# tsurumeso/vocal-remover

Hardware: AMD Instinct MI355X
Metric: spectrogram-frames/sec (inference, CascadedNet n_fft=2048) (higher is better)
Workload: dtype f32; 1 GPU; configs[1]: 30 s stereo 44.1 kHz synthetic song, STFT -> 11 crops of 256 frames in one device batch -> predict_mask -> stitch -> mask apply -> iSTFT x2; n_fft=2048, hop=1024, cropsize=256, parallelism=replicas x1 (songs shard, no collective), input_residency=inputs resident in HBM when the timed region starts

## Files before the change

vocal-remover_amd/csrc/conv_mfma.hip:

```cpp
#include <cstdlib>

#include "conv_stage.h"
#include "kernels.h"

namespace vr {

template <int KS, int S, int DH, int DW, int MT, int TH, int TW, int CK, int WAVES_M>
struct ConvCfg {
    static constexpr int KK = KS * KS;
    static constexpr int WAVES_N = 4 / WAVES_M;
    static constexpr int NG = TH * TW / 32;
    static constexpr int WM = MT / 32 / WAVES_M;
    static constexpr int WN = NG / WAVES_N;
    static constexpr int TH_in = (TH - 1) * S + (KS - 1) * DH + 1;
    static constexpr int TW_in = (TW - 1) * S + (KS - 1) * DW + 1;
    static constexpr int TWp = (TW == 16) ? ((TW_in + 15) / 32 * 32 + 16) : ((TW_in + 1) & ~1);
    static constexpr int XS = CK * TH_in * TWp;
    static constexpr int WS = KK * CK * MT;
    static constexpr int STG = StageGeom<TH_in, TW_in>::TAB + StageGeom<TH_in, TW_in>::SCR;
    static constexpr int LDS_BYTES = (XS + WS + STG) * 4;
    static_assert(WM >= 1 && WN >= 1 && WM * WAVES_M * 32 == MT && WN * WAVES_N == NG, "tile split");
    static_assert(XS % 4 == 0, "weight slab must stay 16B aligned");
    static_assert(TWp >= TW_in, "pitch");
};
// ... 247 lines not shown
}

bool ws_pick(const ConvArgs& a, const ConvShape& s, int* MT_out, int* TH_out);
bool thin16_pick(const ConvArgs& a, const ConvShape& s, int* TH);
void thin16_fill_tiling(ConvArgs& a, int TH);
void thin16_launch_conv(const ConvArgs& a, const ConvShape& s, int TH, hipStream_t st);
bool wino_pick(const ConvArgs& a, const ConvShape& s, int* MT_out);
void wino_fill_tiling(ConvArgs& a, int MT);
void wino_launch_conv(const ConvArgs& a, int MT, hipStream_t st);
struct DmaTile { int MT, TH, TW; };
bool dma_pick(const ConvArgs& a, const ConvShape& s, DmaTile* t);
void dma_fill_tiling(ConvArgs& a, const DmaTile& t);
void dma_launch_conv(const ConvArgs& a, const ConvShape& s, const DmaTile& t, hipStream_t st);
void ws_fill_tiling(ConvArgs& a, int MT, int TH);
void ws_launch_conv(const ConvArgs& a, const ConvShape& s, int MT, int TH, hipStream_t st);

void conv_fill_tiling(ConvArgs& a, const ConvShape& s) {
    int wmt, wth;
    int wino_mt, thin_th;
    if (a.w_hi == 0 && thin16_pick(a, s, &thin_th)) { thin16_fill_tiling(a, thin_th); return; }
    X3Tile x3t;
    if (x3_pick(a, s, &x3t)) { x3_fill_tiling(a, x3t); return; }
    int x3d_mt;
    if (x3d_pick(a, s, &x3d_mt)) { x3d_fill_tiling(a, x3d_mt); return; }
    X3Tile x3st;
    if (x3s_pick(a, s, &x3st)) { x3s_fill_tiling(a, x3st); return; }
    if (wino_pick(a, s, &wino_mt)) { wino_fill_tiling(a, wino_mt); return; }
    DmaTile dt;
    if (dma_pick(a, s, &dt)) { dma_fill_tiling(a, dt); return; }
    if (ws_pick(a, s, &wmt, &wth)) { ws_fill_tiling(a, wmt, wth); return; }
    TileChoice t = pick_tile(a, s);
    a.tiles_w = (a.Wout + t.TW - 1) / t.TW;
    a.tiles_h = (a.Hout + t.TH - 1) / t.TH;
    a.npt = a.N * a.tiles_h * a.tiles_w;
    a.nct = a.CoutPad / t.MT;
}

size_t conv_part_count(const ConvArgs& a, const ConvShape& s) {
    ConvArgs b = a;
    conv_fill_tiling(b, s);
    return (size_t)b.npt;
}

template <int KS, int S, int DH, int DW, int MT, int TH, int TW, int CK, int WAVES_M>
static void launch_inst(const ConvArgs& a, hipStream_t st) {
    using Cfg = ConvCfg<KS, S, DH, DW, MT, TH, TW, CK, WAVES_M>;
    auto kern = conv_mfma_kernel<KS, S, DH, DW, MT, TH, TW, CK, WAVES_M>;
    static std::atomic<unsigned long long> attr_done{0};
    ensure_lds_attr(attr_done, reinterpret_cast<const void*>(kern), Cfg::LDS_BYTES);
    const int groups = (a.npt + 7) / 8;
    const int grid = groups * 8 * a.nct;
    VR_LAUNCH(kern, dim3(grid), dim3(256), Cfg::LDS_BYTES, st, a);
    VR_HIP(hipGetLastError());
}

template <int KS, int S, int DH, int DW, int CK>
static void launch_by_tile(const ConvArgs& a, const TileChoice& t, hipStream_t st) {
    if (t.TW == 32) {
        if constexpr (DH == 1 && DW == 1) {
            if (t.MT == 64) launch_inst<KS, S, DH, DW, 64, 8, 32, CK, 1>(a, st);
            else if (t.TH == 16) {
                if constexpr (S == 1) launch_inst<KS, S, DH, DW, 32, 16, 32, CK, 1>(a, st);
                else throw Error(-2, "16x32 tiles are stride-1 only");
            }
            else            launch_inst<KS, S, DH, DW, 32, 8, 32, CK, 1>(a, st);
        } else {
            throw Error(-2, "dilated conv uses TW=16 tiles only");
        }
    } else {
        if (t.MT == 64) launch_inst<KS, S, DH, DW, 64, 16, 16, CK, 1>(a, st);
        else            launch_inst<KS, S, DH, DW, 32, 16, 16, CK, 1>(a, st);
    }
}

double launch_conv(const ConvArgs& a_in, const ConvShape& s, hipStream_t st) {
    ConvArgs a = a_in;
    static const int dbg = getenv("VR_CONV_DBG") ? atoi(getenv("VR_CONV_DBG")) : 0;
    a.dbg = dbg;
    if (a.w_hi > 0) {
        X3Tile x3t;
        VR_CHECK(a.bf16 == 3 && a.nsrc >= 1 && a.nsrc <= 3 && a.w_lo >= 0 && a.w_lo < a.w_hi && !a.part && x3_pick(a, s, &x3t), -2,
                 "conv column window: only conv_x3h (mfma_mode 3, eval) takes one");
    }
    for (int i = 0; i < a.nsrc && i < 3; ++i) {
        const ConvSrc& c = a.src[i];
        VR_CHECK(!(c.up && c.aff1 && c.aff1 != c.aff0 && c.hsplit < c.H), -2, "conv: an upsampled source cannot carry a row-split affine (hsplit)");
    }
    {
        int wmt, wth;
        int wino_mt, thin_th;
        if (a.w_hi == 0 && a.nsrc >= 1 && a.nsrc <= 3 && thin16_pick(a, s, &thin_th)) {
            thin16_fill_tiling(a, thin_th);
            thin16_launch_conv(a, s, thin_th, st);
            return 2.0 * a.N * (double)a.Hout * a.Wout * (double)a.Cout * a.Cin * s.KS * s.KS;
        }
        X3Tile x3t;
        if (a.nsrc >= 1 && a.nsrc <= 3 && x3_pick(a, s, &x3t)) {
            x3_fill_tiling(a, x3t);
            x3_launch_conv(a, x3t, st);
            return 2.0 * a.N * (double)a.Hout * a.Wout * (double)a.Cout * a.Cin * s.KS * s.KS;
        }
        int x3d_mt;
        if (a.nsrc >= 1 && a.nsrc <= 3 && x3d_pick(a, s, &x3d_mt)) {
            x3d_fill_tiling(a, x3d_mt);
            x3d_launch_conv(a, s, x3d_mt, st);
            return 2.0 * a.N * (double)a.Hout * a.Wout * (double)a.Cout * a.Cin * s.KS * s.KS;
        }
        X3Tile x3st;
        if (x3s_pick(a, s, &x3st)) {
            x3s_fill_tiling(a, x3st);
            x3s_launch_conv(a, x3st, st);
            return 2.0 * a.N * (double)a.Hout * a.Wout * (double)a.Cout * a.Cin * s.KS * s.KS;
        }
        if (a.nsrc >= 1 && a.nsrc <= 3 && wino_pick(a, s, &wino_mt)) {
            wino_fill_tiling(a, wino_mt);
            wino_launch_conv(a, wino_mt, st);
            return 2.0 * a.N * (double)a.Hout * a.Wout * (double)a.Cout * a.Cin * s.KS * s.KS;
        }
        DmaTile dt;
        if (dma_pick(a, s, &dt)) {
            VR_CHECK(a.nsrc >= 1 && a.nsrc <= 3, -2, "conv takes 1..3 sources");
            dma_fill_tiling(a, dt);
            dma_launch_conv(a, s, dt, st);
            return 2.0 * a.N * (double)a.Hout * a.Wout * (double)a.Cout * a.Cin * s.KS * s.KS;
        }
        VR_CHECK(a.tapmask == 0, -2, "a tap-masked conv needs the LDS-DMA kernel (conv_dma_eligible)");
        if (ws_pick(a, s, &wmt, &wth)) {
            VR_CHECK(a.nsrc >= 1 && a.nsrc <= 3, -2, "conv takes 1..3 sources");
            ws_fill_tiling(a, wmt, wth);
            ws_launch_conv(a, s, wmt, wth, st);
            return 2.0 * a.N * (double)a.Hout * a.Wout * (double)a.Cout * a.Cin * s.KS * s.KS;
        }
    }
    conv_fill_tiling(a, s);
    TileChoice t = pick_tile(a, s);
    VR_CHECK(a.CoutPad % t.MT == 0 && a.CoutPad % 32 == 0, -2, "CoutPad must be a multiple of the cout tile");
    VR_CHECK(a.nsrc >= 1 && a.nsrc <= 3, -2, "conv takes 1..3 sources");
    if (s.KS == 1) {
        VR_CHECK(s.stride == 1 && s.dil_h == 1 && s.dil_w == 1, -2, "1x1 conv: stride/dilation must be 1");
        launch_by_tile<1, 1, 1, 1, 32>(a, t, st);
    } else if (s.KS == 3 && s.stride == 1 && s.dil_h == 1 && s.dil_w == 1) {
        launch_by_tile<3, 1, 1, 1, 8>(a, t, st);
    } else if (s.KS == 3 && s.stride == 2 && s.dil_h == 1 && s.dil_w == 1) {
        launch_by_tile<3, 2, 1, 1, 4>(a, t, st);
    } else if (s.KS == 3 && s.stride == 1 && s.dil_h == 4 && s.dil_w == 2) {
        launch_by_tile<3, 1, 4, 2, 4>(a, t, st);
    } else if (s.KS == 3 && s.stride == 1 && s.dil_h == 8 && s.dil_w == 4) {
        launch_by_tile<3, 1, 8, 4, 4>(a, t, st);
    } else if (s.KS == 3 && s.stride == 1 && s.dil_h == 12 && s.dil_w == 6) {
        launch_by_tile<3, 1, 12, 6, 4>(a, t, st);
    } else {
        throw Error(-2, "unsupported conv shape (kernel/stride/dilation)");
    }
    return 2.0 * a.N * (double)a.Hout * a.Wout * (double)a.Cout * a.Cin * s.KS * s.KS;
}

}
```

vocal-remover_amd/csrc/conv_x3h.hip:

```cpp
#include <cstdlib>
#include <type_traits>

#include "conv_epilogue.h"
#include "conv_stage.h"
#include "kernels.h"
#include "lds_dma.h"
#include "x3h_common.h"

namespace vr {

template <int MT, int TH, bool UP = true>
struct X3hCfg {
    static constexpr int TW = 32, CK = 8, KK = 9;
    static constexpr int TH_in = TH + 2, PW = TW + 2;
    static constexpr int NSLOT = TH_in * PW;
    static constexpr int NPASS = (NSLOT + 255) / 256;
    static constexpr int WM = MT / 32, WN = TH / 4;
    static constexpr int PLANE = NSLOT * 16;
    static constexpr int P_BYTES = 2 * PLANE;
    static constexpr int NWP = KK * 2 * MT;
    static constexpr int W_BYTES = NWP * 16;
    static constexpr int NWPASS = (NWP + 255) / 256;
    static constexpr int LROWS = TH / 2 + 3, LW = 20, LSLOT = LROWS * LW;
    static constexpr int L_OFF = P_BYTES + 2 * W_BYTES;
    static constexpr int L_BYTES = UP ? CK * LSLOT * 4 : 0;
    static constexpr int E_OFF = L_OFF + L_BYTES;
    static constexpr int M_OFF = E_OFF + 4 * MT * 4;
    static constexpr int LDS_BYTES = M_OFF + 16;
    static constexpr int OCC = (MT == 32 && TH == 8) ? 3 : 2;
    static constexpr int NXL = 8 * NPASS, NWMIN = (NWP / 64) / 4;
    static constexpr int NG = 14;
    static_assert(TH % 4 == 0 && MT % 32 == 0 && LDS_BYTES <= 80 * 1024 && 2 * NXL + NWMIN < 64 && NXL <= 30 && LSLOT <= 256, "tile");
};

__device__ long long g_x3h_trace[4 * 4 * 6 * 8];
void x3h_trace_read(long long* host, int n) {
    VR_HIP(hipMemcpyFromSymbol(host, HIP_SYMBOL(g_x3h_trace), sizeof(long long) * (size_t)(n < 768 ? n : 768)));
}
void x3h_trace_clear() {
    static long long zeros[768] = {0};
    VR_HIP(hipMemcpyToSymbol(HIP_SYMBOL(g_x3h_trace), zeros, sizeof zeros));
}

template <int MT, int TH, bool UP, bool HI, bool TRACE = false>
__global__ __launch_bounds__(256, (X3hCfg<MT, TH>::OCC + (HI ? 1 : 0))) void conv_x3h_kernel(const ConvArgs a) {
    using Cfg = X3hCfg<MT, TH, UP>;
    constexpr int TW = Cfg::TW, KK = Cfg::KK, PW = Cfg::PW, NSLOT = Cfg::NSLOT, NPASS = Cfg::NPASS, WM = Cfg::WM, WN = Cfg::WN,
                  PLANE = Cfg::PLANE, NWP = Cfg::NWP, NWPASS = Cfg::NWPASS;
    extern __shared__ __attribute__((aligned(16))) char smem_x3h[];
    char* const Pb = smem_x3h;

    const int id = blockIdx.x;
    const int xcd = id & 7;
    const int rr = id >> 3;
    const int ct = rr % a.nct;
    const int per_xcd = (a.npt + 7) >> 3;
    const int pt = (a.dbg & 16) ? (rr / a.nct) * 8 + xcd : xcd * per_xcd + rr / a.nct;
    if (pt >= a.npt) return;
    const int tiles_per_img = a.tiles_h * a.tiles_w;
    const int n = pt / tiles_per_img;
    const int trem = pt - n * tiles_per_img;
    const int h0 = (trem / a.tiles_w) * TH;
    const int w0 = (a.wt0 + trem % a.tiles_w) * TW;
    const int co0 = ct * MT;
    const int tid = threadIdx.x;
    const int lane = tid & 63;
    const int wave = __builtin_amdgcn_readfirstlane(tid >> 6);
    const int nchunk = (a.Cin + 7) >> 3;
    const unsigned lds0 = (unsigned)(size_t)smem_x3h;
    const int dbg = a.dbg & 15;
    const bool prio = (a.dbg & 32) != 0;
    const int trace_wg = TRACE ? (int)blockIdx.x - (int)(gridDim.x / 2) : -1;
    auto stamp = [&](int k, int point) {
        if (TRACE && trace_wg >= 0 && trace_wg < 4 && k >= 2 && k < 8) {
            const long long t = __builtin_readcyclecounter();
            if (lane == 0) g_x3h_trace[((trace_wg * 4 + wave) * 6 + (k - 2)) * 8 + point] = t;
        }
    };

    auto pixel_offset = [&](int p, unsigned sH4) -> int {
        const int s = p * 256 + tid;
        const int r = s / PW, c = s - r * PW;
        const int hi = h0 - 1 + r, wi = w0 - 1 + c;
        const bool ok = s < NSLOT && hi >= 0 && hi < a.Hin && wi >= 0 && wi < a.Win;
        return ok ? (int)((unsigned)hi * sH4 + (unsigned)(wi * 4)) : (int)0x80000000u;
    };
    const ConvSrc& us = a.src[0].up ? a.src[0] : (a.src[1].up ? a.src[1] : a.src[2]);
    constexpr bool any_up = UP;
    int lrow = 0, lcol4 = 0;
    int lidx[NPASS], lstep[NPASS];
    float lh[NPASS], lw_[NPASS];
    if (any_up) {
        const int lr0 = (int)(us.rh * (float)(h0 > 0 ? h0 - 1 : 0)), lc0 = (int)(us.rw * (float)(w0 > 0 ? w0 - 1 : 0));
        const int lr = lr0 + tid / Cfg::LW, lc = lc0 + tid % Cfg::LW;
        const bool lok = tid < Cfg::LSLOT && lr < us.H && lc < us.W;
        lrow = lok ? lr : 0;
        lcol4 = lok ? lc * 4 : (int)0x80000000u;
#pragma unroll
        for (int p = 0; p < NPASS; ++p) {
            const int s = p * 256 + tid;
            const int r = s / PW, c = s - r * PW;
            const int hi = h0 - 1 + r, wi = w0 - 1 + c;
            const bool ok = s < NSLOT && hi >= 0 && hi < a.Hin && wi >= 0 && wi < a.Win;
            const float h1r = us.rh * (float)(ok ? hi : 0), w1r = us.rw * (float)(ok ? wi : 0);
            const int h1 = (int)h1r, w1 = (int)w1r;
            lidx[p] = ok ? ((h1 - lr0) * Cfg::LW + (w1 - lc0)) * 32 : -1;
            const int rs = (h1 + 1 < us.H && h1 + 1 - lr0 < Cfg::LROWS) ? Cfg::LW * 32 : 0;
            const int cs = (w1 + 1 < us.W && w1 + 1 - lc0 < Cfg::LW) ? 32 : 0;
            lstep[p] = (rs << 16) | cs;
            lh[p] = h1r - (float)h1;
            lw_[p] = w1r - (float)w1;
        }
    }
    unsigned woff0;
    {
        const int q = wave * 64 + lane;
        const int m = q % MT, tp = q / MT;
        woff0 = (unsigned)((tp * a.CoutPad + m) * 16);
    }
    const unsigned wstep = (unsigned)((256 / MT) * a.CoutPad * 16);
    const long long wchunk_bytes = (long long)KK * 2 * a.CoutPad * 16;
    auto issue_w = [&](int k) {
        const char* wb = static_cast<const char*>(a.x3w) + k * wchunk_bytes + (long long)co0 * 16;
        const i32x4 wr = make_rsrc(reinterpret_cast<const float*>(wb), (unsigned)(wchunk_bytes - (long long)co0 * 16));
        const unsigned ws_b = lds0 + (unsigned)(Cfg::P_BYTES + (k & 1) * Cfg::W_BYTES);
#pragma unroll
        for (int i = 0; i < NWPASS; ++i) {
            const int pp = wave + 4 * i;
            if ((pp + 1) * 64 <= NWP) dma16s(ws_b + pp * 1024, woff0, wr, (unsigned)i * wstep);
// ... 71 lines not shown
    };
    auto read_max_exp = [&]() -> int {
        const vr_i32x4 mm = *reinterpret_cast<const vr_i32x4*>(smem_x3h + Cfg::M_OFF);
        const int w = max(max(mm[0], mm[1]), max(mm[2], mm[3]));
        return __builtin_amdgcn_readfirstlane(w) >> 23;
    };
    auto convert = [&](auto par) {
        constexpr int PAR = decltype(par)::value;
#pragma unroll
        for (int p = 0; p < NPASS; ++p) {
            const int s = p * 256 + tid;
            if ((p + 1) * 256 <= NSLOT || s < NSLOT) {
                vr_i32x4 ph, pl;
                if (upm[PAR] != 0u) {
                    const char* lq = smem_x3h + Cfg::L_OFF + (lidx[p] >= 0 ? lidx[p] : 0);
                    const int rs = lstep[p] >> 16, cs = lstep[p] & 0xffff;
                    const float h1l = lh[p], h0l = 1.f - h1l, w1l = lw_[p], w0l = 1.f - w1l;
                    if (upm[PAR] == 0xFFu) {
                        vr_f32x4h nb[4][2];
#pragma unroll
                        for (int q4 = 0; q4 < 4; ++q4)
#pragma unroll
                            for (int hf = 0; hf < 2; ++hf)
                                nb[q4][hf] = *reinterpret_cast<const vr_f32x4h*>(lq + (q4 >> 1) * rs + (q4 & 1) * cs + hf * 16);
#pragma unroll
                        for (int cl = 0; cl < 8; ++cl) {
                            const float v00 = nb[0][cl >> 2][cl & 3], v01 = nb[1][cl >> 2][cl & 3], v10 = nb[2][cl >> 2][cl & 3], v11 = nb[3][cl >> 2][cl & 3];
                            const float v = h0l * (w0l * v00 + w1l * v01) + h1l * (w0l * v10 + w1l * v11);
                            xr[PAR][p][cl] = lidx[p] >= 0 ? v : 0.f;
                        }
                    } else {
#pragma unroll
                        for (int cl = 0; cl < 8; ++cl) {
                            if ((upm[PAR] >> cl) & 1u) {
                                const char* q = lq + cl * 4;
                                const float v00 = *reinterpret_cast<const float*>(q), v01 = *reinterpret_cast<const float*>(q + cs),
                                            v10 = *reinterpret_cast<const float*>(q + rs), v11 = *reinterpret_cast<const float*>(q + rs + cs);
                                const float v = h0l * (w0l * v00 + w1l * v01) + h1l * (w0l * v10 + w1l * v11);
                                xr[PAR][p][cl] = lidx[p] >= 0 ? v : 0.f;
                            }
                        }
                    }
                }
#pragma unroll
                for (int j = 0; j < 4; ++j) {
                    int h, l;
                    split2h_pair(xr[PAR][p][2 * j], xr[PAR][p][2 * j + 1], psc, h, l);
                    ph[j] = h; pl[j] = l;
                }
                char* q = Pb + s * 16;
                *reinterpret_cast<vr_i32x4*>(q) = ph;
                *reinterpret_cast<vr_i32x4*>(q + PLANE) = pl;
            }
        }
    };

    const int khalf = lane >> 5, l31 = lane & 31;
    const int bq = (wave * WN * PW + l31) * 16;
    const int bX = bq + khalf * PLANE, bY1 = bq + khalf * 16, bY2 = bq + khalf * (PW - 2) * 16;
    const int aX = l31 * 16, aY = (MT + l31 + khalf * 2 * MT) * 16;

    f32x16 acc[WM][WN];
#pragma unroll
    for (int mi = 0; mi < WM; ++mi)
#pragma unroll
        for (int ni = 0; ni < WN; ++ni)
#pragma unroll
            for (int r = 0; r < 16; ++r) acc[mi][ni][r] = 0.f;

    using P0 = std::integral_constant<int, 0>;
    using P1 = std::integral_constant<int, 1>;
    float ecv[4];
    {
        const int ec = co0 + (tid & (MT - 1));
        const int ecc = ec < a.Cout ? ec : a.Cout - 1;
        const i32x4 rb = make_rsrc(a.bias, a.bias ? 0x7FFFFFF0u : 0u);
        const i32x4 re = make_rsrc(a.epi, a.epi ? 0x7FFFFFF0u : 0u);
        const i32x4 rw = make_rsrc(reinterpret_cast<const float*>(static_cast<const char*>(a.x3w) + nchunk * wchunk_bytes), 0x7FFFFFF0u);
        ecv[0] = x3h_load(rb, ecc * 4);
        ecv[1] = x3h_load(re, ecc * 8);
        ecv[2] = x3h_load(re, ecc * 8 + 4);
        ecv[3] = x3h_load(rw, ec * 4);
    }
    auto follow = [&](int e, bool first) {
        const int need = 140 - (e < 14 ? 14 : e);
        shlo = (first || need < shlo) ? need : shlo;
        int nsh = sh;
        if (first || need < sh - 1) nsh = need;
        else if (need > sh + 12) {
            nsh = need < sh + 64 ? need : sh + 64;
            nsh = nsh < shlo + 64 ? nsh : shlo + 64;
            nsh = nsh > sh ? nsh : sh;
        }
        if (nsh != sh) {
            if (!first) {
                const int d = nsh - sh;
                const float f = d < -126 ? 0.f : x3h_pow2(d);
#pragma unroll
                for (int mi = 0; mi < WM; ++mi)
#pragma unroll
                    for (int ni = 0; ni < WN; ++ni)
#pragma unroll
                        for (int r = 0; r < 16; ++r) acc[mi][ni][r] *= f;
            }
            sh = nsh;
            psc = x3h_pow2(sh);
        }
    };
#pragma unroll
    for (int cl = 0; cl < 8; ++cl) load_channel(0, cl, P0{});
    issue_w(0);
#pragma unroll
    for (int cl = 0; cl < 8; ++cl) load_channel(1, cl, P1{});
    wait_pixels(P0{}, std::integral_constant<int, Cfg::NXL + Cfg::NWMIN>{});
    asm volatile("; landed %0 %1 %2 %3" : "+v"(ecv[0]), "+v"(ecv[1]), "+v"(ecv[2]), "+v"(ecv[3]));
    if (tid < MT) {
        float* E = reinterpret_cast<float*>(smem_x3h + Cfg::E_OFF);
        E[tid] = ecv[0];
        E[MT + tid] = a.epi ? ecv[1] : 1.f;
        E[2 * MT + tid] = a.epi ? ecv[2] : 0.f;
        E[3 * MT + tid] = ecv[3];
    }
    post_max(P0{});
    if (any_up) stage_lowres(P0{});
    lds_barrier();
    follow(read_max_exp(), true);
    convert(P0{});
    asm volatile("s_waitcnt vmcnt(%0) lgkmcnt(0)" :: "n"(Cfg::NXL) : "memory");
    __builtin_amdgcn_s_barrier();
    asm volatile("" ::: "memory");

    auto chunk = [&](int k, auto par) {
        constexpr int PAR = decltype(par)::value;
        const bool more = k + 1 < nchunk;
        stamp(k, 0);
        {
            const char* Wb = smem_x3h + Cfg::P_BYTES + PAR * Cfg::W_BYTES;
            vr_f16x8 A[2][WM], B[2][WN];
            auto read_group = [&](int g, int buf) {
                const bool isY = g == 13 || (g < 12 && g % 3 == 2);
                const int t = g >= 12 ? 8 : 2 * (g / 3) + (g % 3 == 1 ? 1 : 0);
                const int ty = t / 3, tx = t % 3;
#pragma unroll
                for (int mi = 0; mi < WM; ++mi) {
                    const char* q = Wb + (t * 2 * MT + mi * 32) * 16;
                    if (!isY) A[buf][mi] = *reinterpret_cast<const vr_f16x8*>(q + aX);
                    else if (t < 8) A[buf][mi] = *reinterpret_cast<const vr_f16x8*>(q + aY);
                    else {
                        const vr_i32x4 v = *reinterpret_cast<const vr_i32x4*>(q + aX + MT * 16);
                        vr_i32x4 z;
#pragma unroll
                        for (int j = 0; j < 4; ++j) z[j] = khalf ? 0 : v[j];
                        A[buf][mi] = __builtin_bit_cast(vr_f16x8, z);
                    }
                }
#pragma unroll
                for (int ni = 0; ni < WN; ++ni) {
                    const int o = ((ni + ty) * PW + tx) * 16;
                    if (!isY) B[buf][ni] = *reinterpret_cast<const vr_f16x8*>(Pb + bX + o);
                    else if (t == 8) B[buf][ni] = *reinterpret_cast<const vr_f16x8*>(Pb + bq + o);
                    else if (t == 2) B[buf][ni] = *reinterpret_cast<const vr_f16x8*>(Pb + bY2 + o);
                    else B[buf][ni] = *reinterpret_cast<const vr_f16x8*>(Pb + bY1 + o);
                }
            };
            auto mfma_group = [&](int buf) {
#pragma unroll
                for (int mi = 0; mi < WM; ++mi)
#pragma unroll
                    for (int ni = 0; ni < WN; ++ni) acc[mi][ni] = mfma_f16x16(A[buf][mi], B[buf][ni], acc[mi][ni]);
            };
            read_group(0, 0);
            if (prio) __builtin_amdgcn_s_setprio(1);
#pragma unroll
            for (int g = 0; g < Cfg::NG; ++g) {
                const int cur = g & 1;
                if (g + 1 < Cfg::NG) read_group(g + 1, cur ^ 1);
                if (more) {
                    if (g == 0) issue_w(k + 1);
                    if (g >= 1 && g <= 4) { load_channel(k + 2, 2 * g - 2, par); load_channel(k + 2, 2 * g - 1, par); }
                }
                __builtin_amdgcn_sched_barrier(0);
                mfma_group(cur);
                __builtin_amdgcn_sched_barrier(0);
            }
            if (prio) __builtin_amdgcn_s_setprio(0);
        }
        stamp(k, 1);
        if (more) {
            using Q = std::integral_constant<int, PAR ^ 1>;
            wait_pixels(Q{}, std::integral_constant<int, Cfg::NXL + Cfg::NWMIN>{});
            stamp(k, 2);
            post_max(Q{});
            if (any_up) stage_lowres(Q{});
            stamp(k, 3);
            lds_barrier();
            stamp(k, 4);
            follow(read_max_exp(), false);
            if (dbg != 3) convert(Q{});
            stamp(k, 5);
            asm volatile("s_waitcnt vmcnt(%0) lgkmcnt(0)" :: "n"(Cfg::NXL) : "memory");
            stamp(k, 6);
            __builtin_amdgcn_s_barrier();
            asm volatile("" ::: "memory");
            stamp(k, 7);
        }
    };
    for (int k = 0; k < nchunk; k += 2) {
        chunk(k, P0{});
        if (k + 1 < nchunk) chunk(k + 1, P1{});
    }
    asm volatile("s_waitcnt vmcnt(0)" ::: "memory");

    if (dbg == 4) return;
    {
        const float fo = x3h_pow2(-sh);
        const float* Wi = reinterpret_cast<const float*>(smem_x3h + Cfg::E_OFF) + 3 * MT;
#pragma unroll
        for (int mi = 0; mi < WM; ++mi)
#pragma unroll
            for (int rq = 0; rq < 4; ++rq) {
                const vr_f32x4h wi = *reinterpret_cast<const vr_f32x4h*>(Wi + mi * 32 + 8 * rq + 4 * khalf);
#pragma unroll
                for (int ni = 0; ni < WN; ++ni)
#pragma unroll
                    for (int j = 0; j < 4; ++j) acc[mi][ni][rq * 4 + j] = (acc[mi][ni][rq * 4 + j] * fo) * wi[j];
            }
    }
    {
        int hon[WN], won[WN];
#pragma unroll
        for (int ni = 0; ni < WN; ++ni) { hon[ni] = h0 + wave * WN + ni; won[ni] = w0 + l31; }
        epi_store<MT, WM, WN>(VR_EPI_ARGS(a), acc, reinterpret_cast<const float*>(smem_x3h + Cfg::E_OFF), n, co0, khalf,
                              h0 + TH <= a.Hout && w0 + TW <= a.Wout, hon, won);
    }
    if (a.part) {
        __syncthreads();
        float* red = reinterpret_cast<float*>(smem_x3h);
#pragma unroll
        for (int mi = 0; mi < WM; ++mi) {
#pragma unroll
            for (int r = 0; r < 16; ++r) {
                float s1 = 0.f, s2 = 0.f;
#pragma unroll
                for (int ni = 0; ni < WN; ++ni) {
                    const int ho = h0 + wave * WN + ni, wo = w0 + l31;
                    if (ho < a.Hout && wo < a.Wout) {
                        const float v = acc[mi][ni][r];
                        s1 += v;
                        s2 = fmaf(v, v, s2);
                    }
                }
                s1 = half_wave_sum_dpp(s1);
                s2 = half_wave_sum_dpp(s2);
                if (l31 == 16) {
                    const int m = mi * 32 + (r & 3) + 8 * (r >> 2) + 4 * khalf;
                    red[(wave * MT + m) * 2 + 0] = s1;
                    red[(wave * MT + m) * 2 + 1] = s2;
                }
            }
        }
        __syncthreads();
        if (tid < MT) {
            float s1 = 0.f, s2 = 0.f;
#pragma unroll
            for (int w = 0; w < 4; ++w) {
                s1 += red[(w * MT + tid) * 2 + 0];
                s2 += red[(w * MT + tid) * 2 + 1];
            }
            const int co = co0 + tid;
            if (co < a.Cout) {
                a.part[((long long)pt * a.Cout + co) * 2 + 0] = s1;
                a.part[((long long)pt * a.Cout + co) * 2 + 1] = s2;
            }
        }
    }
}

__device__ __forceinline__ float* x3h_tail(void* o, int Cin, int KK, int CoutPad) {
    return reinterpret_cast<float*>(static_cast<char*>(o) + (size_t)((Cin + 7) / 8) * KK * 2 * CoutPad * 16);
}
__device__ __forceinline__ void x3h_wscale_block(const float* __restrict__ w, void* o, int Cin, int KK, int CoutPad, int cb) {
    __shared__ float red[8][32];
    if (cb * 32 >= CoutPad) return;
    const int c = threadIdx.x & 31, g = threadIdx.x >> 5, co = cb * 32 + c;
    const int rows = Cin * KK;
    float m = 0.f;
    for (int r = g; r < rows; r += 8) m = fmaxf(m, fabsf(w[(long long)r * CoutPad + co]));
    red[g][c] = m;
    __syncthreads();
    if (g == 0) {
#pragma unroll
        for (int j = 1; j < 8; ++j) m = fmaxf(m, red[j][c]);
        int e = __float_as_int(m) >> 23;
        e = e < 15 ? 15 : (e > 254 ? 254 : e);
        float* t = x3h_tail(o, Cin, KK, CoutPad);
        t[co] = __int_as_float((e - 14) << 23);
        t[CoutPad + co] = __int_as_float((268 - e) << 23);
    }
}
__device__ __forceinline__ void x3h_weights_elem(const float* __restrict__ w, void* o, int Cin, int KK, int CoutPad, long long gid) {
    const int cin8 = (Cin + 7) / 8 * 8;
    if (gid >= (long long)cin8 * KK * CoutPad) return;
    const int co = (int)(gid % CoutPad);
    const int t = (int)((gid / CoutPad) % KK);
    const int ci = (int)(gid / ((long long)CoutPad * KK));
    const float sc = x3h_tail(o, Cin, KK, CoutPad)[CoutPad + co];
    const float v = ci < Cin ? w[((long long)ci * KK + t) * CoutPad + co] : 0.f;
    const _Float16 h1 = (_Float16)(v * sc);
    const _Float16 h2 = (_Float16)fmaf(v, sc, -(float)h1);
    _Float16* q = static_cast<_Float16*>(o) + ((((long long)(ci >> 3) * KK + t) * 2) * CoutPad + co) * 8 + (ci & 7);
    q[0] = h1;
    q[(long long)CoutPad * 8] = h2;
}
__global__ void x3h_wscale_kernel(const float* __restrict__ w, void* o, int Cin, int KK, int CoutPad) {
    x3h_wscale_block(w, o, Cin, KK, CoutPad, blockIdx.x);
}
__global__ void x3h_weights_kernel(const float* __restrict__ w, void* o, int Cin, int KK, int CoutPad) {
    x3h_weights_elem(w, o, Cin, KK, CoutPad, (long long)blockIdx.x * blockDim.x + threadIdx.x);
}
__global__ void x3h_wscale_batched_kernel(const X3WDesc* __restrict__ d) {
    const X3WDesc e = d[blockIdx.y];
    x3h_wscale_block(e.w, e.o, e.Cin, e.KK, e.CoutPad, blockIdx.x);
}
__global__ void x3h_weights_batched_kernel(const X3WDesc* __restrict__ d) {
    const X3WDesc e = d[blockIdx.y];
    x3h_weights_elem(e.w, e.o, e.Cin, e.KK, e.CoutPad, (long long)blockIdx.x * blockDim.x + threadIdx.x);
}

void launch_x3h_weights(const float* w, void* o, int Cin, int KK, int CoutPad, hipStream_t st) {
    const long long n = (long long)((Cin + 7) / 8 * 8) * KK * CoutPad;
    VR_LAUNCH(x3h_wscale_kernel, dim3((unsigned)((CoutPad + 31) / 32)), dim3(256), 0, st, w, o, Cin, KK, CoutPad);
    VR_LAUNCH(x3h_weights_kernel, dim3((unsigned)((n + 255) / 256)), dim3(256), 0, st, w, o, Cin, KK, CoutPad);
    VR_HIP(hipGetLastError());
}
void launch_x3h_weights_batched(const X3WDesc* d_descs, int n, long long max_elems, int max_cout_pad, hipStream_t st) {
    if (n <= 0) return;
    VR_LAUNCH(x3h_wscale_batched_kernel, dim3((unsigned)((max_cout_pad + 31) / 32), (unsigned)n), dim3(256), 0, st, d_descs);
    VR_LAUNCH(x3h_weights_batched_kernel, dim3((unsigned)((max_elems + 255) / 256), (unsigned)n), dim3(256), 0, st, d_descs);
    VR_HIP(hipGetLastError());
}

template <int MT, int TH, bool UP, bool HI, bool TRACE = false>
static void x3h_launch_up(const ConvArgs& a, hipStream_t st) {
    using Cfg = X3hCfg<MT, TH, UP>;
    auto kern = conv_x3h_kernel<MT, TH, UP, HI, TRACE>;
    static std::atomic<unsigned long long> attr_done{0};
    ensure_lds_attr(attr_done, reinterpret_cast<const void*>(kern), Cfg::LDS_BYTES);
    const int groups = (a.npt + 7) / 8;
    VR_LAUNCH(kern, dim3(groups * 8 * a.nct), dim3(256), Cfg::LDS_BYTES, st, a);
    VR_HIP(hipGetLastError());
}

template <int MT, int TH>
static void x3h_launch(const ConvArgs& a, hipStream_t st) {
    static const int hi = [] { const char* e = getenv("VR_X3H_HI"); return e ? atoi(e) : 0; }();
    if (a.dbg & 64) {
        if (a.src[0].up | a.src[1].up | a.src[2].up) x3h_launch_up<MT, TH, true, false, true>(a, st);
        else x3h_launch_up<MT, TH, false, false, true>(a, st);
        return;
    }
    if (a.src[0].up | a.src[1].up | a.src[2].up) x3h_launch_up<MT, TH, true, false>(a, st);
    else if (hi && TH == 8) x3h_launch_up<MT, TH, false, (TH == 8)>(a, st);
    else x3h_launch_up<MT, TH, false, false>(a, st);
}

void x3h_launch_conv(const ConvArgs& a, const X3Tile& t, hipStream_t st) {
    if (t.MT == 64) x3h_launch<64, 8>(a, st);
    else if (t.TH == 16) x3h_launch<32, 16>(a, st);
    else x3h_launch<32, 8>(a, st);
}

}
```

vocal-remover_amd/csrc/debug.hip:

```cpp
#include <cmath>
#include <cstdlib>
#include <cstring>
#include <memory>
#include <string>
#include <vector>

#include "model.h"

namespace vr {

namespace {

struct DevBuf {
    float* p = nullptr;
    size_t n = 0;
    DevBuf() = default;
    explicit DevBuf(size_t n_) : n(n_) {
        VR_HIP(hipMalloc(&p, (n ? n : 1) * sizeof(float)));
        VR_HIP(hipMemset(p, 0, (n ? n : 1) * sizeof(float)));
        VR_HIP(hipStreamSynchronize(nullptr));
    }
    DevBuf(const float* host, size_t n_) : n(n_) {
        VR_HIP(hipMalloc(&p, (n ? n : 1) * sizeof(float)));
        if (host && n) VR_HIP(hipMemcpy(p, host, n * sizeof(float), hipMemcpyHostToDevice));
// ... 245 lines not shown
    ConvArgs a{};
    a.nsrc = nsrc; a.N = N; a.Cout = Cout; a.CoutPad = (Cout + 31) / 32 * 32;
    a.w_lo = (int)dims[8]; a.w_hi = (int)dims[9]; a.d1 = (int)dims[10]; a.d2 = (int)dims[11];
    a.bf16 = mfma_mode;
    a.pad_h = KS == 1 ? 0 : dh; a.pad_w = KS == 1 ? 0 : dw;
    std::vector<std::unique_ptr<DevBuf>> keep;
    auto upload = [&](const float* host, size_t n) { keep.emplace_back(new DevBuf(host, n)); return keep.back()->p; };
    int Cin = 0;
    const ConvSrc* ups = nullptr;
    for (int i = 0; i < nsrc; ++i) {
        const int64_t* d = dims + 12 + 10 * i;
        const float* const* si = in + 3 + 4 * i;
        Tensor t;
        t.N = N; t.C = (int)d[0]; t.H = (int)d[1]; t.W = (int)d[2];
        const bool up = d[3] != 0;
        t.hsplit = (int)d[4];
        const size_t floats = (size_t)d[5];
        t.sN = d[7]; t.sC = d[8]; t.sH = d[9];
        VR_CHECK(si[0] && view_fits(d[6], t.sN, t.sC, t.sH, N, t.C, t.H, t.W, floats), -2, who + "a source view leaves its buffer");
        t.p = upload(si[0], floats) + d[6];
        t.slope = fp[1 + i];
        if (si[1]) t.aff0 = upload(si[1], (size_t)t.C * 2);
        if (si[2]) t.aff1 = upload(si[2], (size_t)t.C * 2);
        if (si[3]) t.post = upload(si[3], (size_t)N * t.C);
        a.src[i] = make_src(t, up, 0);
        const int vh = up ? 2 * t.H : t.H, vw = up ? 2 * t.W : t.W;
        if (i == 0) { a.Hin = vh; a.Win = vw; }
        VR_CHECK(vh == a.Hin && vw == a.Win, -2, who + "the sources must share the input size");
        if (up && ups) VR_CHECK(ups->H == t.H && ups->W == t.W && ups->sH == t.sH, -2, who + "upsampled sources must share H, W and row stride");
        if (up) ups = &a.src[i];
        Cin += t.C;
        if (i == 0) a.c1 = Cin;
        if (i <= 1) a.c2 = Cin;
    }
    a.Cin = Cin;
    a.Hout = a.Hin; a.Wout = a.Win;
    const int KK = KS * KS;
    std::vector<float> wk((size_t)Cin * KK * a.CoutPad, 0.f);
    for (int co = 0; co < Cout; ++co)
        for (int ci = 0; ci < Cin; ++ci)
            for (int k = 0; k < KK; ++k) wk[((size_t)ci * KK + k) * a.CoutPad + co] = in[0][((size_t)co * Cin + ci) * KK + k];
    DevBuf dwk(wk.data(), wk.size());
    a.w = dwk.p;
    if (in[1]) a.bias = upload(in[1], (size_t)Cout);
    if (in[2]) { a.epi = upload(in[2], (size_t)Cout * 2); a.epi_slope = fp[0]; }
    DebugWeightForms wf;
    debug_weight_forms(dwk.p, Cin, KS, 1, dh, dw, a.CoutPad, a.Win, transformed, a, wf);
    std::vector<std::unique_ptr<GuardedBuf>> dst(3);
    const int c1 = a.d1 < Cout ? a.d1 : Cout, c2 = a.d2 < Cout ? a.d2 : Cout;
    VR_CHECK(0 <= c1 && c1 <= c2, -2, who + "need 0 <= d1 <= d2");
    const int seg_c[3] = {c1, c2 - c1, Cout - c2};
    for (int i = 0; i < ndst; ++i) {
        const int64_t* d = dims + 12 + 10 * nsrc + 7 * i;
        const float* host = in[3 + 4 * nsrc + i];
        if (!d[0]) continue;
        VR_CHECK(host && out[i], -2, who + "a present destination needs its buffer, in and out");
        VR_CHECK(seg_c[i] == 0 || view_fits(d[3], d[4], d[5], d[6], N, seg_c[i], a.Hout, a.Wout, (size_t)d[2]), -2,
                 who + "a destination view leaves its buffer");
        dst[i].reset(new GuardedBuf(host, (size_t)d[2]));
        a.dst[i] = ConvDst{dst[i]->p() + d[3], d[4], d[5], d[6], d[1] != 0 ? 1 : 0, 0};
    }
    const ConvShape shp{KS, 1, dh, dw};
    size_t npt = 0;
    std::unique_ptr<DevBuf> part;
    if (want_part) { npt = conv_part_count(a, shp); part.reset(new DevBuf(npt * Cout * 2)); a.part = part->p; }
    launch_conv(a, shp, stream);
    VR_HIP(hipStreamSynchronize(stream));
    for (int i = 0; i < ndst; ++i)
        if (dst[i]) {
            VR_CHECK(dst[i]->intact(), -3, who + "the launch stored outside a destination's buffer");
            dst[i]->download(out[i]);
        }
    if (want_part) {
        std::vector<float> ph(npt * Cout * 2);
        part->download(ph.data());
        for (int c = 0; c < Cout; ++c) {
            double s1 = 0, s2 = 0;
            for (size_t i = 0; i < npt; ++i) { s1 += ph[(i * Cout + c) * 2]; s2 += ph[(i * Cout + c) * 2 + 1]; }
            out[ndst][2 * c] = (float)s1; out[ndst][2 * c + 1] = (float)s2;
        }
    }
}

void Model::debug_wgrad_launch(const int64_t* dims, int ndims, const float* fp, int nfp, const float* const* in, int nin, float* const* out,
                               int nout) {
    const std::string who = "vr_debug_kernel(wgrad_launch): ";
    VR_CHECK(ndims >= 13 && nfp >= 3 && nin >= 2 && nout >= 2, -2, who + "too few arguments");
    const int nsrc = (int)dims[0], N = (int)dims[1], Cout = (int)dims[2], KS = (int)dims[3], stride = (int)dims[4];
    const int dh = (int)dims[5], dw = (int)dims[6], flags = (int)dims[7];
    const bool batch_as_h = flags & 1, accumulate = flags & 2, defer = flags & 4, twice = flags & 8, accumulate2 = flags & 16;
    VR_CHECK(nsrc >= 1 && nsrc <= 3 && N >= 1 && Cout >= 1 && (KS == 1 || KS == 3) && (stride == 1 || stride == 2) && dh >= 1 && dw >= 1, -2,
             who + "1..3 sources, a 1x1 or 3x3 kernel, stride 1 or 2");
    VR_CHECK(ndims >= 13 + 10 * nsrc && nin >= 2 + 4 * nsrc, -2, who + "too few arguments");
    VR_CHECK(in[0] && in[1] && out[0] && out[1], -2, who + "missing dz, gradient or an output");
    WgradArgs w{};
    ConvArgs& a = w.in;
    a.nsrc = nsrc; a.Cout = Cout; a.CoutPad = (Cout + 31) / 32 * 32;
    a.d1 = a.d2 = 1 << 30;
    a.pad_h = KS == 1 ? 0 : dh; a.pad_w = KS == 1 ? 0 : dw;
    std::vector<std::unique_ptr<DevBuf>> keep;
    auto upload = [&](const float* host, size_t n) { keep.emplace_back(new DevBuf(host, n)); return keep.back()->p; };
    int Cin = 0, Hin = 0, Win = 0;
    const ConvSrc* ups = nullptr;
    for (int i = 0; i < nsrc; ++i) {
        const int64_t* d = dims + 13 + 10 * i;
        const float* const* si = in + 2 + 4 * i;
        Tensor t;
        t.N = N; t.C = (int)d[0]; t.H = (int)d[1]; t.W = (int)d[2];
        const bool up = d[3] != 0;
        t.hsplit = (int)d[4];
        const size_t floats = (size_t)d[5];
        t.sN = d[7]; t.sC = d[8]; t.sH = d[9];
        VR_CHECK(si[0] && view_fits(d[6], t.sN, t.sC, t.sH, N, t.C, t.H, t.W, floats), -2, who + "a source view leaves its buffer");
        t.p = upload(si[0], floats) + d[6];
        t.slope = fp[i];
        if (si[1]) t.aff0 = upload(si[1], (size_t)t.C * 2);
        if (si[2]) t.aff1 = upload(si[2], (size_t)t.C * 2);
        if (si[3]) t.post = upload(si[3], (size_t)N * t.C);
        a.src[i] = make_src(t, up, 0);
        const int vh = up ? 2 * t.H : t.H, vw = up ? 2 * t.W : t.W;
        if (i == 0) { Hin = vh; Win = vw; }
        VR_CHECK(vh == Hin && vw == Win, -2, who + "the sources must share the input size");
        if (up && ups) VR_CHECK(ups->H == t.H && ups->W == t.W && ups->sH == t.sH, -2, who + "upsampled sources must share H, W and row stride");
        if (up) ups = &a.src[i];
        Cin += t.C;
        if (i == 0) a.c1 = Cin;
        if (i <= 1) a.c2 = Cin;
    }
    a.Cin = Cin;
    if (nsrc < 2) a.c1 = Cin;
    if (nsrc < 3) a.c2 = Cin;
    const int Hout0 = (Hin + 2 * a.pad_h - dh * (KS - 1) - 1) / stride + 1, Wout = (Win + 2 * a.pad_w - dw * (KS - 1) - 1) / stride + 1;
    VR_CHECK(Hout0 >= 1 && Wout >= 1, -2, who + "empty output");
    const size_t zfloats = (size_t)dims[8];
    VR_CHECK(view_fits(dims[9], dims[10], dims[11], dims[12], N, Cout, Hout0, Wout, zfloats), -2, who + "the dz view leaves its buffer");
    DevBuf dz(in[0], zfloats);
    w.dz = dz.p + dims[9];
    int Nk = N;
    if (batch_as_h) {
        VR_CHECK(KS == 1 && Hin == 1, -2, who + "batch-as-rows view needs a 1x1 conv on H=1 input");
        for (int i = 0; i < nsrc; ++i) {
            VR_CHECK(!a.src[i].post && !a.src[i].up, -2, who + "batch-as-rows: unsupported source flags");
            a.src[i].sH = a.src[i].sN; a.src[i].sN = 0; a.src[i].H = N;
        }
        Hin = N; Nk = 1;
        w.zN = 0; w.zC = dims[11]; w.zH = dims[10];
    } else {
        w.zN = dims[10]; w.zC = dims[11]; w.zH = dims[12];
    }
    a.N = Nk; a.Hin = Hin; a.Win = Win;
    a.Hout = (Hin + 2 * a.pad_h - dh * (KS - 1) - 1) / stride + 1; a.Wout = Wout;
    w.Cout = Cout; w.CoutPad = a.CoutPad;
    w.allow_wino = train_wino ? 1 : 0;
    w.bf16 = mfma_mode;
    const ConvShape shp{KS, stride, dh, dw};
    WgradArgs pl = w;
    {
        int CB = 0, MT = 0;
        wgrad_choose(pl, shp, &CB, &MT);
    }
    const size_t gfloats = (size_t)Cin * KS * KS * a.CoutPad, sfloats = wgrad_scratch_floats(w, shp);
    VR_CHECK((size_t)pl.P * (size_t)pl.part_stride <= sfloats, -4, who + "the plan's slabs exceed wgrad_scratch_floats");
    GuardedBuf grad(in[1], gfloats);
    const std::vector<float> nans(sfloats, std::nanf(""));
    GuardedBuf scratch(nans.data(), sfloats), scratch2(twice ? nans.data() : nullptr, twice ? sfloats : 0);
    w.part = scratch.p();
// ... 93 lines not shown
    debug_dgrad_weight_forms(P, KS, stride, dh, dw, forms);
    struct WsRestore {
        Model* m; Arena saved;
        ~WsRestore() { m->ws = saved; m->dry = false; }
    } ws_restore{this, ws};
    ws.dry = true; ws.base = nullptr; ws.off = 0; ws.peak = 0; dry = true;
    bwd_conv_dgrad(r, f);
    dry = false;
    const size_t wfloats = (ws.peak + 3) / 4;
    const std::vector<float> nans(wfloats, std::nanf(""));
    GuardedBuf wsbuf(nans.data(), wfloats);
    ws = Arena{};
    ws.base = reinterpret_cast<char*>(wsbuf.p()); ws.cap = wfloats * 4;
    int path = DG_NONE;
    try {
        path = bwd_conv_dgrad(r, f);
    } catch (...) {
        (void)hipStreamSynchronize(stream);
        for (int i = 0; i < nsrc; ++i) grads[i]->download(out[i]);
        throw;
    }
    VR_HIP(hipStreamSynchronize(stream));
    bool intact = wsbuf.intact();
    for (int i = 0; i < nsrc; ++i) intact = intact && grads[i]->intact();
    VR_CHECK(intact, -3, who + "the launch stored outside a gradient buffer or the workspace");
    for (int i = 0; i < nsrc; ++i) grads[i]->download(out[i]);
    const int64_t info[4] = {path, (int64_t)wfloats, 0, 0};
    std::memcpy(out[nsrc], info, sizeof info);
}

void Model::debug_wgrad_reduce(const int64_t* dims, int ndims, const float* const* in, int nin, float* const* out, int nout) {
    const std::string who = "vr_debug_kernel(wgrad_reduce): ";
    VR_CHECK(ndims >= 1, -2, who + "too few arguments");
    const int nd = (int)dims[0];
    VR_CHECK(nd >= 1 && nd <= 128 && ndims >= 1 + 6 * nd && nin >= 2 * nd && nout >= 2 * nd + 1, -2, who + "1..128 descriptors, six dims each");
    std::vector<std::unique_ptr<DevBuf>> slabs;
    std::vector<std::unique_ptr<GuardedBuf>> o_imm, o_bat;
    std::vector<WgReduceDesc> descs;
    for (int j = 0; j < nd; ++j) {
        const int64_t* d = dims + 1 + 6 * j;
        const long long P = d[0], n = d[1], stride = d[2], floats = d[4], off = d[5];
        VR_CHECK(P >= 1 && n >= 1 && stride >= n && off >= 0 && off + n <= floats, -2, who + "need P, n >= 1, stride >= n and the output inside its buffer");
        VR_CHECK(in[2 * j] && in[2 * j + 1] && out[2 * j] && out[2 * j + 1] && out[2 * nd], -2, who + "missing buffer");
        slabs.emplace_back(new DevBuf(in[2 * j], (size_t)(P * stride)));
        o_imm.emplace_back(new GuardedBuf(in[2 * j + 1], (size_t)floats));
        o_bat.emplace_back(new GuardedBuf(in[2 * j + 1], (size_t)floats));
        descs.push_back(WgReduceDesc{slabs.back()->p, stride, o_bat.back()->p() + off, n, (int)P, d[3] != 0 ? 1 : 0, 0});
    }
    for (int j = 0; j < nd; ++j) {
        const WgReduceDesc& d = descs[j];
        launch_wgrad_reduce(d.part, d.stride, d.P, o_imm[j]->p() + dims[1 + 6 * j + 5], d.n, d.accumulate, stream);
    }
    const int vec = wgrad_reduce_vec(descs.data(), nd);
    wred_host = descs;
    flush_wgrad_sums();
    VR_HIP(hipStreamSynchronize(stream));
    for (int j = 0; j < nd; ++j) {
        VR_CHECK(o_imm[j]->intact() && o_bat[j]->intact(), -3, who + "a slab sum stored outside its output buffer");
        o_imm[j]->download(out[2 * j]);
        o_bat[j]->download(out[2 * j + 1]);
    }
    out[2 * nd][0] = (float)vec;
}

void Model::debug_kernel(const std::string& name, const int64_t* dims, int ndims, const float* fp, int nfp,
                         const float* const* in, int nin, float* const* out, int nout) {
    DeviceGuard dev_guard(device);
    auto need = [&](int nd, int nf, int ni, int no) {
        VR_CHECK(ndims >= nd && nfp >= nf && nin >= ni && nout >= no, -2, "vr_debug_kernel(" + name + "): too few arguments");
    };
    hipStream_t st = stream;
    if (name == "x3h_trace") {
        need(1, 0, 0, dims[0] ? 1 : 0);
        VR_HIP(hipDeviceSynchronize());
        if (!dims[0]) { x3h_trace_clear(); return; }
        long long raw[768];
        x3h_trace_read(raw, 768);
        long long lo = 0;
        for (long long v : raw) if (v && (!lo || v < lo)) lo = v;
        for (int i = 0; i < 768; ++i) out[0][i] = raw[i] ? (float)(raw[i] - lo) : -1.f;
        return;
    }
    if (name == "conv_launch") { debug_conv_launch(dims, ndims, fp, nfp, in, nin, out, nout); return; }
    if (name == "wgrad_launch") { debug_wgrad_launch(dims, ndims, fp, nfp, in, nin, out, nout); return; }
    if (name == "wgrad_reduce") { debug_wgrad_reduce(dims, ndims, in, nin, out, nout); return; }
    if (name == "dgrad_launch") { debug_dgrad_launch(dims, ndims, in, nin, out, nout); return; }
    if (name == "tensor_pass") { debug_tensor_pass(dims, ndims, fp, nfp, in, nin, out, nout); return; }
    if (name == "weight_forms") { debug_weight_form_launch(dims, ndims, in, nin, out, nout); return; }
    if (name == "layer_forms") { debug_layer_forms(dims, ndims, out, nout); return; }
    if (name == "bn_backward") {
        need(4, 3, 7, 6);
        const int N = (int)dims[0], C = (int)dims[1], H = (int)dims[2], W = (int)dims[3];
        const bool view = ndims >= 10;
        const long long off = view ? dims[5] : 0, sH = view ? dims[8] : W, sC = view ? dims[7] : (long long)H * W, sN = view ? dims[6] : sC * C;
        const size_t n = view ? (size_t)dims[4] : (size_t)N * C * H * W;
        const int aff_bcast = view && dims[9] != 0 ? 1 : 0;
        VR_CHECK(N >= 1 && C >= 1 && H >= 1 && W >= 1, -2, "bn_backward: empty tensor");
        VR_CHECK(view_fits(off, sN, sC, sH, N, C, H, W, n), -2, "bn_backward: the view leaves its buffer");
        VR_CHECK(!aff_bcast || C == 1, -2, "bn_backward: a broadcast affine table belongs to a single-channel BatchNorm");
        DevBuf z(in[0], n), gamma(in[2], C), beta(in[3], C), rm(in[5], C), rv(in[6], C);
        GuardedBuf g(in[1], n);
        DevBuf post(in[4], in[4] ? (size_t)N * C : 0);
        std::vector<float> part((size_t)C * 2);
        for (int c = 0; c < C; ++c) {
            double s1 = 0, s2 = 0;
            for (int b = 0; b < N; ++b)
                for (int h = 0; h < H; ++h) {
                    const float* q = in[0] + off + b * sN + c * sC + h * sH;
                    for (int i = 0; i < W; ++i) { s1 += q[i]; s2 += (double)q[i] * q[i]; }
                }
            part[2 * c] = (float)s1; part[2 * c + 1] = (float)s2;
        }
        const int bcast_rows = aff_bcast ? 8 : 0;
        DevBuf dpart(part.data(), part.size()), aff((size_t)(aff_bcast ? bcast_rows : C) * 2), smean(C), sinv(C), dgamma(C), dbeta(C);
        BNFinalizeArgs f{};
        f.part = dpart.p; f.nparts = 1; f.pstride = C * 2; f.count = (double)N * H * W;
        f.w = gamma.p; f.b = beta.p; f.rm = rm.p; f.rv = rv.p; f.affine = aff.p; f.save_mean = smean.p; f.save_invstd = sinv.p;
        f.C = C; f.eps = fp[1]; f.momentum = fp[2]; f.broadcast = bcast_rows;
        launch_bn_finalize(f, st);
        BnBwdArgs a{};
        a.g = g.p() + off; a.z = z.p + off; a.N = N; a.C = C; a.H = H; a.W = W; a.sH = sH; a.sC = sC; a.sN = sN;
        a.aff = aff.p; a.aff_bcast = aff_bcast; a.slope = fp[0]; a.post = in[4] ? post.p : nullptr;
        a.gamma = gamma.p; a.save_mean = smean.p; a.save_invstd = sinv.p; a.dgamma = dgamma.p; a.dbeta = dbeta.p; a.acc_grads = 1;
        DevBuf coef((size_t)C * 3), bpart((size_t)bn_bwd_chunks(a) * C * 2);
        a.coef = coef.p; a.part = bpart.p;
        launch_bn_bwd(a, st);
        VR_HIP(hipStreamSynchronize(st));
        VR_CHECK(g.intact(), -3, "bn_backward: a store outside the gradient's buffer");
        g.download(out[0]); dgamma.download(out[1]); dbeta.download(out[2]); rm.download(out[4]); rv.download(out[5]);
        if (out[3]) VR_HIP(hipMemcpy(out[3], aff.p, (size_t)C * 2 * sizeof(float), hipMemcpyDeviceToHost));
    } else if (name == "lstm") {
        const int flags = ndims >= 4 ? (int)dims[3] : 0;
        const bool infer = flags & 1, bwd_only = flags & 2;
        need(3, 0, infer ? 3 : 4, infer ? 1 : 4);
        const int N = (int)dims[0], T = (int)dims[1], H = (int)dims[2], G = 4 * H;
        VR_CHECK(N > 0 && T > 0 && H > 0, -2, "lstm: N, T, H must be positive");
        DevBuf gx(in[0], (size_t)N * 2 * G * T), wf(in[1], (size_t)G * H), wr(in[2], (size_t)G * H), h((size_t)N * 2 * H * T);
        if (infer) {
            launch_bilstm(gx.p, wf.p, wr.p, h.p, N, T, H, st);
            VR_HIP(hipStreamSynchronize(st));
            h.download(out[0]);
            return;
        }
        DevBuf dh(in[3], (size_t)N * 2 * H * T), save((size_t)N * 2 * T * 5 * H), dgx((size_t)N * 2 * G * T);
        const float* f0 = nin >= 5 ? in[4] : nullptr;
        const float* r0 = nin >= 6 ? in[5] : nullptr;
        std::vector<float> zeros(f0 && r0 ? 0 : (size_t)G * H, 0.f);
        DevBuf dwf(f0 ? f0 : zeros.data(), (size_t)G * H), dwr(r0 ? r0 : zeros.data(), (size_t)G * H);
        if (!bwd_only) launch_bilstm_train(gx.p, wf.p, wr.p, h.p, save.p, N, T, H, st);
        launch_bilstm_bwd(dh.p, save.p, wf.p, wr.p, dgx.p, N, T, H, st);
        DevBuf wpart(lstm_whh_grad_scratch_floats(N, H));
        launch_lstm_whh_grad(dgx.p, h.p, dwf.p, dwr.p, N, T, H, 1, wpart.p, st);
        VR_HIP(hipStreamSynchronize(st));
        h.download(out[0]); dgx.download(out[1]); dwf.download(out[2]); dwr.download(out[3]);
    } else if (name == "upsample") {
        need(4, 0, 2, 2);
        const int N = (int)dims[0], C = (int)dims[1], H = (int)dims[2], W = (int)dims[3];
        const size_t n = (size_t)N * C * H * W;
        const bool view = ndims >= 10;
        const long long off = view ? dims[5] : 0, gN = view ? dims[6] : (long long)C * H * W, gC = view ? dims[7] : (long long)H * W, gH = view ? dims[8] : W;
        const size_t gfloats = view ? (size_t)dims[4] : n;
        VR_CHECK(N >= 1 && C >= 1 && H >= 1 && W >= 1, -2, "upsample: empty tensor");
        VR_CHECK(!view || (nin >= 3 && in[2]), -2, "upsample: a strided gradient needs its backing buffer");
        VR_CHECK(view_fits(off, gN, gC, gH, N, C, H, W, gfloats), -2, "upsample: the gradient view leaves its buffer");
        const std::vector<float> zeros(view ? 0 : n, 0.f);
        DevBuf x(in[0], n), dhi(in[1], 4 * n), up(4 * n);
// ... 416 lines not shown
```

vocal-remover_amd/csrc/kernels.h:

```cpp
#pragma once
#include "vr_common.h"

namespace vr {

struct HeadDst {
    float* p;
    long long dN, dC, dH;
    int w_lo, w_hi;
    int pad_rows;
    float* const* items;
    const int* item_pitch;
};
void launch_head_sigmoid(const Tensor& x, const float* w , const HeadDst& d, hipStream_t st);
void launch_head_complex(const Tensor& x, const float* w , const HeadDst& d, hipStream_t st);
int launch_squeeze_conv(const Tensor& x, const float* w , float* out, float* part, bool dry, hipStream_t st,
                        const float* epi = nullptr);

void launch_avgpool_h(const Tensor& x, float* out, hipStream_t st);

struct BNFoldDesc { const float *w, *b, *rm, *rv; float* affine; int C; int bcast; };
void launch_bn_fold_eval(const BNFoldDesc* d_descs, int ndesc, int maxC, float eps, hipStream_t st);
struct BNFinalizeArgs {
    const float* part; int nparts; int pstride;
    double count;
    const float *w, *b; float *rm, *rv;
    float* affine; float* save_mean; float* save_invstd;
    int C; float eps, momentum;
    int broadcast;
};
void launch_bn_finalize(const BNFinalizeArgs& a, hipStream_t st);

void launch_rows_affine_relu(const float* x, float* out, const float* aff, int N, int R, int W, hipStream_t st);

void launch_add(const float* a, const float* b, float* out, int n, hipStream_t st);

void launch_materialize(const Tensor& x, float* out, hipStream_t st);
struct AugDesc { float coef, coef_mix, lam; int flags; };
void launch_augment(const float2* X, const float2* Y, const float2* Xi, const float2* Yi, const AugDesc* desc, const float* rw,
                    int B, int T, int bins, float* Xmag, float* Ymag, bool out_complex, hipStream_t st);
struct AugCrops { const float2 *X, *y, *X_mix, *y_mix; };
void launch_augment_resident(const AugCrops* table, const AugDesc* desc, const float* rw, int B, int T, int bins, float* Xmag,
                             float* Ymag, bool out_complex, hipStream_t st);
bool thin16_pick(const ConvArgs& a, const ConvShape& s, int* TH);
void thin16_fill_tiling(ConvArgs& a, int TH);
void thin16_launch_conv(const ConvArgs& a, const ConvShape& s, int TH, hipStream_t st);
bool s2d_fused_eligible(const ConvArgs& a);
void launch_s2d_fused(const ConvArgs& a, hipStream_t st);
struct S2WDesc { const float* w; float* wc; int Cin, Cout, CoutPad, CinPad; };
void launch_s2_class_weights(const S2WDesc* d_descs, int n, long long max_elems, hipStream_t st);
void launch_wino_weights(const float* w, float* u, int Cin, int CoutPad, hipStream_t st);
struct WinoWDesc { const float* w; void* u; int Cin, CoutPad; };
void launch_wino_weights_batched(const WinoWDesc* d_descs, int n, long long max_elems, bool split6, hipStream_t st);
size_t wino_weights6_bytes(int Cin, int CoutPad);
void launch_wino_weights6(const float* w, void* u6, int Cin, int CoutPad, hipStream_t st);
struct X3Tile { int MT, TH; };
struct X3WDesc { const float* w; void* o; int Cin, KK, CoutPad; };
bool x3_pick(const ConvArgs& a, const ConvShape& s, X3Tile* t);
void x3_fill_tiling(ConvArgs& a, const X3Tile& t);
void x3_launch_conv(const ConvArgs& a, const X3Tile& t, hipStream_t st);
size_t x3_weights_bytes(int Cin, int KK, int CoutPad);
void launch_x3_weights(const float* w, void* o, int Cin, int KK, int CoutPad, hipStream_t st);
void launch_x3_weights_batched(const X3WDesc* d_descs, int n, long long max_elems, hipStream_t st);
void x3h_launch_conv(const ConvArgs& a, const X3Tile& t, hipStream_t st);
void x3h_trace_read(long long* host, int n);
void x3h_trace_clear();
void launch_x3h_weights(const float* w, void* o, int Cin, int KK, int CoutPad, hipStream_t st);
void launch_x3h_weights_batched(const X3WDesc* d_descs, int n, long long max_elems, int max_cout_pad, hipStream_t st);
bool x3d_pick(const ConvArgs& a, const ConvShape& s, int* MT);
void x3d_fill_tiling(ConvArgs& a, int MT);
void x3d_launch_conv(const ConvArgs& a, const ConvShape& s, int MT, hipStream_t st);
bool x3d_aspp_eligible(const ConvArgs* c4, const ConvShape* s4);
void x3d_launch_aspp(const ConvArgs* c4, hipStream_t st);
bool x3s_pick(const ConvArgs& a, const ConvShape& s, X3Tile* t);
void x3s_fill_tiling(ConvArgs& a, const X3Tile& t);
void x3s_launch_conv(const ConvArgs& a, const X3Tile& t, hipStream_t st);
void launch_upsample2x(const Tensor& x, float* out, hipStream_t st);

void launch_bilstm(const float* gx, const float* whh_f, const float* whh_r, float* out,
                   int N, int T, int H, hipStream_t st);

void launch_bilstm_train(const float* gx, const float* whh_f, const float* whh_r, float* out, float* save,
                         int N, int T, int H, hipStream_t st);
void launch_bilstm_bwd(const float* dh, const float* save, const float* whh_f, const float* whh_r, float* dgx,
                       int N, int T, int H, hipStream_t st);
size_t lstm_whh_grad_scratch_floats(int N, int H);
void launch_lstm_whh_grad(const float* dgx, const float* hout, float* dwhh_f, float* dwhh_r, int N, int T, int H,
                          int accumulate, float* part, hipStream_t st);

struct BnBwdArgs {
    float* g;
    const float* z;
    int N, C, H, W;
    long long sN, sC, sH;
    const float* aff;
    int aff_bcast;
    float slope;
    const float* post;
    const float *gamma, *save_mean, *save_invstd;
    float *dgamma, *dbeta;
    int acc_grads;
    float* coef;
    float* part;
};
int bn_bwd_chunks(const BnBwdArgs& a);
void launch_bn_bwd(const BnBwdArgs& a, hipStream_t st);

void launch_upsample_bwd(const float* dhi, int N, int C, int H, int W, float* glo, long long gN, long long gC,
                         long long gH, int accumulate, hipStream_t st);
void launch_sum_h(const float* d, int N, int C, int H, int W, float* out, hipStream_t st);
void launch_avgpool_bwd(const float* gp, float* g, int N, int C, int H, int W, long long sN, long long sC, long long sH,
                        int accumulate, hipStream_t st);
void launch_thin_dgrad(const Tensor& x, int CO, const float* w, const float* dz, float* g, int accumulate, hipStream_t st);
int thin_wgrad_blocks(const Tensor& x);
void launch_thin_wgrad(const Tensor& x, int CO, const float* dz, float* part, float* dw, int accumulate, hipStream_t st);
void launch_reduce_rows(const float* part, long long stride, int P, float* out, long long n, int accumulate, float scale,
                        hipStream_t st);
int head_loss_blocks(const Tensor& x);
void launch_head_loss(const Tensor& x, const float* w, const float* X, const float* Y, int bins, float gscale,
                      float* dlogit, float* mask_out, float* loss_part, float* loss_out, float loss_scale, hipStream_t st);
void launch_head_bwd(const float* dmask, const float* mask, int N, int H, int W, int bins, float* dlogit, hipStream_t st);
void launch_head_loss_complex(const Tensor& x, const float* w, const float* X, const float* Y, int bins, float gscale,
                              float* dlogit, float* mask_out, float* loss_part, float* loss_out, float loss_scale, hipStream_t st);
void launch_head_bwd_complex(const Tensor& x, const float* w, const float* dmask, int bins, float* dlogit, hipStream_t st);
struct MagL1 {};
void launch_head_mag_l1(const Tensor& x, const float* w, const float* X, const float* Y, int bins, float* mask_out, float* loss_part,
                        float* loss_out, float loss_scale, hipStream_t st);
struct FlipDesc { const float* w; float* wt; int Cin, Cout, KK, CinPad, CoutPad; };
void launch_flip_transpose(const FlipDesc* d_descs, int n, hipStream_t st);
void launch_adam(float* p, const float* g, float* m, float* v, long long n, double lr, double b1, double b2, double eps,
                 long long step, double gscale, hipStream_t st);
void launch_channel_sum(const float* d, int N, int C, int W, float* out, int accumulate, hipStream_t st);
void launch_f32_to_bf16(const float* x, unsigned short* y, long long n, hipStream_t st);
void launch_bf16_to_f32(const unsigned short* x, float* y, long long n, hipStream_t st);

void launch_mul_crop(const float* x, float* m, bool cplx, long long rows, int T, int Wm, int off, hipStream_t st);
int l1_crop_blocks();
enum L1CropForm { L1_CROP_REAL = 0, L1_CROP_COMPLEX = 1, L1_CROP_MAG = 2 };
void launch_l1_crop(L1CropForm form, const float* pred, const float* y, long long rows, int T, int Wm, int off, float* part, float* loss,
                    hipStream_t st);

struct FFTPlan { int n_fft; int log2n; float2* twiddle; float* window; };
void launch_stft(const FFTPlan& pl, const float* wave, long long L, int hop, int T, float2* spec, hipStream_t st);
void launch_istft(const FFTPlan& pl, const float2* spec, int hop, int T, float* frames, float* wave, hipStream_t st);
bool istft_masked_available(const FFTPlan& pl, int hop);
void launch_istft_masked(const FFTPlan& pl, const float2* spec, int hop, int T, const float* mask_a, int Wa, const float* mask_b,
                         int Wb, int shift, const float* wgt, int which, float* wave, hipStream_t st);
// ... 161 lines not shown
```

vocal-remover_amd/csrc/model.h:

```cpp
#pragma once
#include <chrono>
#include <deque>
#include <functional>
#include <map>
#include <memory>
#include <string>
#include <vector>

#include "kernels.h"

namespace vr {

struct Arena {
    char* base = nullptr;
    size_t cap = 0, off = 0, peak = 0;
    bool dry = false;
    void* alloc(size_t bytes) {
        const size_t a = (off + 255) & ~size_t(255);
        off = a + bytes;
        if (off > peak) peak = off;
        if (dry) return reinterpret_cast<void*>(uintptr_t(256));
        if (off > cap) throw Error(-4, "workspace arena overflow (planning bug)");
        return base + a;
    }
// ... 97 lines not shown
    long long bytes = 0;
    ResidentSet(int device, int bins);
    ~ResidentSet();
    ResidentSet(const ResidentSet&) = delete;
    ResidentSet& operator=(const ResidentSet&) = delete;
    int add(const float* X, const float* y, long long rows);
private:
    static constexpr size_t kPiece = size_t(8) << 20;
    hipStream_t up = nullptr;
    char* stage[2] = {nullptr, nullptr};
    hipEvent_t drained[2] = {nullptr, nullptr};
    void upload(float2* dst, const float* src, size_t n_bytes);
};

struct HeadScratch {
    float *dlogit, *lpart, *wpart;
    float *mask, *dmask, *wave[3], *part, *table;
};
struct TrainHead {
    int kind; bool cplx;
    const float *w, *X, *Y; int bins;
    float* mask;
    float* loss;
    float loss_scale, grad_scale, sdr_scale;
    float* g; int g_acc; float* dw; int dw_acc;
};
template <class ALLOC>
HeadScratch head_scratch(ALLOC&& allocf, const FFTPlan& pl, int hop, const Tensor& f3, int kind, bool cplx, int bins) {
    const int CO = cplx ? 4 : 2;
    HeadScratch s{};
    s.dlogit = allocf((size_t)f3.N * CO * f3.H * f3.W);
    s.lpart = allocf((size_t)head_loss_blocks(f3));
    s.wpart = allocf((size_t)thin_wgrad_blocks(f3) * CO * f3.C);
    if (kind == 0) return s;
    const WaveTermFloats wf = wave_term_floats(pl, hop, kind, f3.N * 2, f3.W);
    s.mask = allocf((size_t)f3.N * 2 * bins * f3.W * 2);
    s.dmask = allocf((size_t)f3.N * 2 * bins * f3.W * 2);
    for (int i = 0; i < wf.waves; ++i) s.wave[i] = allocf(wf.wave);
    s.part = allocf(wf.part);
    s.table = allocf(wf.table);
    return s;
}
void run_train_head(const FFTPlan& pl, const Tensor& f3, const TrainHead& h, const HeadScratch& s, WaveTable* staging, hipStream_t st);
void launch_head_grads(const Tensor& f3, int CO, const float* w, const float* dlogit, float* wpart, float* g, int g_acc, float* dw,
                       int dw_acc, hipStream_t st);

class Model {
public:
    Model(int device, int n_fft, int hop, int nout, int nout_lstm, bool is_complex = false);
    ~Model();

    int device, n_fft, hop, nout, nout_lstm, max_bin, output_bin, offset = 64;
    bool is_complex = false;
    bool complex_train = false;
    int loss_kind = 0;
    double sdr_weight = 0.01, last_mag_l1 = 0.0, last_sdr = 0.0;
    bool loss_terms_valid = false;
    WaveTable wave_host{};
    double last_y_sdr = 0.0, last_noise_sdr = 0.0, last_alpha = 0.0;
    void set_loss(int kind, double weight);
    float finish_wave_loss(const float* l4);
    float finish_wsdr_loss(const float* l7);
    int nin = 2;
    void need_real_mask(const char* what) const;
    void need_real_mask_train(const char* what) const;

    std::deque<Param> params;
    std::map<std::string, Param*> by_key;
    void set_param(const std::string& key, const void* host, const int64_t* shape, int ndim);
    void get_param(const std::string& key, void* host, int64_t cap_bytes);
    void set_training(bool t);
    bool training = false;
    bool fwd_only = false;
    bool taping() const { return training && !fwd_only; }

    void forward_api(const float* x, bool x_on_device, int B, int T, int mode, float* out, bool out_on_device);

    void validate_api(const float* X, const float* Y, bool on_dev, int B, int T, float* loss_out);
    void debug_kernel(const std::string& name, const int64_t* dims, int ndims, const float* fp, int nfp,
                      const float* const* in, int nin, float* const* out, int nout);

    void debug_conv_launch(const int64_t* dims, int ndims, const float* fp, int nfp, const float* const* in, int nin, float* const* out,
                           int nout);
    void debug_wgrad_launch(const int64_t* dims, int ndims, const float* fp, int nfp, const float* const* in, int nin, float* const* out,
                            int nout);
    void debug_wgrad_reduce(const int64_t* dims, int ndims, const float* const* in, int nin, float* const* out, int nout);
    void debug_dgrad_launch(const int64_t* dims, int ndims, const float* const* in, int nin, float* const* out, int nout);
    void debug_tensor_pass(const int64_t* dims, int ndims, const float* fp, int nfp, const float* const* in, int nin, float* const* out,
                           int nout);
    void debug_weight_form_launch(const int64_t* dims, int ndims, const float* const* in, int nin, float* const* out, int nout);
    void debug_layer_forms(const int64_t* dims, int ndims, float* const* out, int nout);
    void stft_api(const float* wave, bool on_dev, long long L, float* spec, bool spec_on_dev);
    void istft_api(const float* spec, bool on_dev, int T, float* wave, bool wave_on_dev);
    void separate_run(int n_songs, const float* const* in, bool in_on_dev, const int* T, const long long* L, int tta, int batchsize,
                      int cropsize, float* const* y, float* const* v, bool out_on_dev, const int* pcm_channels = nullptr,
                      const int* pcm_fmt = nullptr, bool solo = false, const EvalArgs* eval = nullptr);
    bool pcm_available() const;
    void check_pcm(const void* bytes, int channels, int fmt, const std::string& who) const;
    void stft_pcm_api(const void* bytes, bool on_dev, long long L, int channels, int fmt, float* spec, bool spec_on_dev);
    void istft_pcm16_api(const float* spec, bool on_dev, int T, int16_t* out, bool out_on_dev);
    void run_crop_chunks(int patches, int bs, const std::function<void(int, int)>& run_crops);
    StreamState* stream_open(int cropsize, int batchsize, int flags, double coef_re, double coef_im);
    void stream_push(StreamState& S, const float* wave, bool on_dev, long long n, bool flush, float* y, float* v, bool out_on_dev,
                     long long capacity, long long* n_out);
    void stream_push_many(int n_streams, StreamState* const* S, const float* const* wave, bool on_dev, const long long* n, const int* flush,
                          int batchsize, float* const* y, float* const* v, bool out_on_dev, const long long* capacity, long long* n_out);
    void stream_close(StreamState* S);
    void arena_bytes(long long* staging, long long* workspace) const { *staging = (long long)io.cap; *workspace = (long long)ws.cap; }

    void debug_conv(const float* x, int N, int Cin, int H, int W, const float* w_oihw, int Cout, int KS, int stride,
                    int dh, int dw, int up, const float* aff, float slope, const float* bias, float* out,
                    float* stats_out);
    struct DebugWeightForms {
        float* wino = nullptr;
        void* wino6 = nullptr;
        void* x3w = nullptr;
        DebugWeightForms() = default;
        ~DebugWeightForms() { (void)hipFree(wino); (void)hipFree(wino6); (void)hipFree(x3w); }
        DebugWeightForms(const DebugWeightForms&) = delete;
        DebugWeightForms& operator=(const DebugWeightForms&) = delete;
    };
    void debug_weight_forms(const float* dw_kmajor, int Cin, int KS, int stride, int dh, int dw, int CoutPad, int Win, bool transformed,
                            ConvArgs& a, DebugWeightForms& f);
    bool record_taps = false;
    std::map<std::string, Tensor> taps;
    int64_t get_tap(const std::string& name, float* host, int64_t cap_floats, int64_t* shape4);

    bool profiling = false;
    LaunchProfiler* launch_prof = nullptr;
    std::string profile_report;
    void profile_begin();
    void augment_api(const float* Xc, const float* yc, const float* Xi, const float* yi, const void* desc, const float* rw,
                     int B, int T, int bins, bool in_on_dev, float* Xmag, float* ymag, bool out_on_dev, bool out_complex = false);
    void dataset_batch_api(const ResidentSet& set, const ResidentCrop* crops, const void* desc, const float* rw, int B, int T,
                           float* Xmag, float* ymag, bool out_on_dev, bool out_complex = false);
    char* aug_buf = nullptr; size_t aug_cap = 0;
    void aug_reserve(size_t need);
    bool train_wino = true;
    int mfma_mode = 3;
    bool x3_mode() const { return mfma_mode == 2 || mfma_mode == 3; }
    int default_mfma_mode = 3;
    bool serial = false;
    bool crop_window = true;
    int net_w_lo = 0, net_w_hi = 0;
    void set_option(const std::string& name, int value);
    void reset_adam_state();
    void profile_end(double* conv_ms, double* conv_flops, double* conv_bytes, int* launches);

    hipStream_t stream = nullptr;
    hipStream_t side_stream = nullptr;
    hipEvent_t ev_fork = nullptr, ev_join = nullptr;
    bool band_fork_active = false;
    bool gs_clear_pending = false;
    bool wgrad_on_side = false;
    struct Lane { hipStream_t main = nullptr, side = nullptr; hipEvent_t fork = nullptr, join = nullptr, start = nullptr, done = nullptr; Arena ws; };
    std::vector<Lane> lanes;
    void swap_lane(int i);

private:
    float* p_arena = nullptr; size_t p_floats = 0;
    float* b_arena = nullptr; size_t b_floats = 0;
    Arena ws;
    Arena io;
    void ensure_ws(size_t bytes);
    int plan_B = -1, plan_T = -1; bool plan_training = false; size_t plan_peak = 0;
    void ensure_io(size_t bytes);

    std::deque<BN> bns;
    std::vector<BN*> bn_list;
    std::vector<Conv*> wino_list;
    struct PendingConv { ConvArgs a; ConvShape shp; double flops, bytes; bool stats; BNFinalizeArgs fin; BN* bn; };
    std::vector<PendingConv>* conv_sink = nullptr;
    int x3d_mode = 2;
    int conv_w_lo = 0, conv_w_hi = 0;
    std::vector<Conv*> x3d_list;
    int x3s_mode = x3s_default();
    static int x3s_default() { const char* e = getenv("VR_CONV_X3S"); return (e && atoi(e) == 0) ? 0 : 1; }
    std::vector<Conv*> x3s_list;
    float* wino_arena = nullptr;
    float* winot_arena = nullptr;
    std::map<const Param*, float*> winot_of;
    char* wino6_arena = nullptr;
    char* winot6_arena = nullptr;
    std::map<const Param*, void*> winot6_of;
    char* x3_arena = nullptr;
    char* x3t_arena = nullptr;
    std::map<const Param*, void*> x3t_of;
    std::map<const Param*, void*> x3dt_of;
    std::vector<WgReduceDesc> wred_host, wred_sent;
    WgReduceDesc* wred_dev = nullptr;
    size_t wred_cap = 0;
    void flush_wgrad_sums();
    struct X3Batch { std::vector<X3WDesc> host; X3WDesc* dev = nullptr; long long max_elems = 0; };
    X3Batch xb_fwd, xb_bwd;
    void run_x3_batch(X3Batch& b, std::vector<X3WDesc>& descs);
    static long long x3_batch_max_elems(const std::vector<X3WDesc>& descs);
    static int x3_batch_max_cout_pad(const std::vector<X3WDesc>& descs);
    static long long wino_batch_max_elems(const std::vector<WinoWDesc>& descs, bool split6);
    static long long s2w_batch_max_elems(const std::vector<S2WDesc>& descs);
    void refresh_wino(bool with_dgrad);
    struct WinoBatch { std::vector<WinoWDesc> host; WinoWDesc* dev = nullptr; long long max_elems = 0; };
    WinoBatch wb_fwd, wb_bwd, wb_fwd6, wb_bwd6;
    void run_wino_batch(WinoBatch& b, std::vector<WinoWDesc>& descs, bool split6);
    BNFoldDesc* d_fold = nullptr;
    bool affine_dirty = true;
    void fold_eval_affines();

    BaseNetL nets_[5];
    Conv tail1, tail2;
    Param *out_w = nullptr, *aux_out_w = nullptr;

    FFTPlan plan{};

    Param* add_param(const std::string& key, std::vector<int64_t> shape, ParamKind kind, bool trainable);
    BN* add_bn(const std::string& prefix, int C, int bcast);
    void build_cba(Conv& L, const std::string& prefix, int nin, int nout_, int ks, int stride, int pad_h, int pad_w,
                   int dh, int dw, float slope);
    void build_basenet(BaseNetL& B, const std::string& prefix, int nin, int c, int nin_lstm, int nout_lstm_);
    void finalize_layout();

    struct SrcSpec { Tensor t; bool up = false; int bcastH = 0; float* plain = nullptr; };
    enum TapeKind { TK_CONV, TK_AVGPOOL, TK_SQUEEZE, TK_LSTM, TK_DENSE_ACT };
    struct TapeRec {
        TapeKind kind;
        Conv* L = nullptr;
        std::vector<SrcSpec> srcs;
// ... 2 lines not shown
        bool batch_as_h = false;
        const float* bias = nullptr;
        Param* bias_param = nullptr;
        LSTMMod* M = nullptr;
        Tensor aux;
        float* save = nullptr;
        float* buf0 = nullptr;
        float* buf1 = nullptr;
        int chain = 0;
    };
    std::vector<TapeRec> tape;
    Arena gs;
    std::vector<std::pair<size_t, size_t>> gs_zero, gs_zero_plan;
    std::map<const float*, bool> g_fresh;
    float* galloc(size_t n, bool plain);
    bool g_first(const float* g);
    void clear_gs_zero_ranges(hipStream_t st);
    float* g_arena = nullptr;
    float* m_arena = nullptr; float* v_arena = nullptr;
    float* wt_arena = nullptr; size_t wt_floats = 0;
    FlipDesc* d_flip = nullptr; int n_flip = 0;
    std::map<const Param*, float*> wt_of;
    float* s2w_arena = nullptr;
    std::map<const Param*, float*> s2w_of;
    std::vector<Conv*> s2_list;
    S2WDesc* d_s2w = nullptr;
    long long s2w_max = 0;
    long long adam_step = 0;
    float* grad_of(const Param* p) { return p->grad_override ? p->grad_override : g_arena + (p->dev - p_arena); }
public:
    void debug_conv_bwd(const float* x, int N, int Cin, int H, int W, const float* w_oihw, int Cout, int KS, int stride,
                        int dh, int dw, int up, const float* aff, float slope, const float* dz, float* dx_out,
                        float* dw_out);
private:
    void ensure_train_state();
    void refresh_train_weights();
    template <class F> void plan_train_arenas(F&& dry_run, size_t extra_ws, bool clear_beside);
    void wait_gs_clear();
    void backward();
    void bwd_conv(TapeRec& r);
    enum DgradPath { DG_NONE = 0, DG_STRIDE1 = 1, DG_S2_FUSED = 2, DG_S2_CLASSES = 3, DG_S2_ZINS = 4 };
    int bwd_conv_dgrad(TapeRec& r, const ConvArgs& f);
    struct DebugDgradForms {
        Model* m = nullptr;
        const Param* P = nullptr;
        float *wt = nullptr, *winot = nullptr, *s2w = nullptr;
        void *x3t = nullptr, *flip_desc = nullptr, *s2_desc = nullptr;
        DebugDgradForms() = default;
        ~DebugDgradForms();
        DebugDgradForms(const DebugDgradForms&) = delete;
        DebugDgradForms& operator=(const DebugDgradForms&) = delete;
    };
    void debug_dgrad_weight_forms(const Param& P, int KS, int stride, int dh, int dw, DebugDgradForms& f);
    void bwd_bn_of(const Tensor& out, Conv& L);
    std::vector<float> dropout_host;
    int dropout_mode = 1;
    unsigned long long dropout_seed = 0x5DEECE66Dull;
    unsigned long long train_calls = 0;
    void prepare_dropout(int B);
    float* dropout_buf = nullptr; size_t dropout_cap = 0;
public:
    void train_fwd_bwd_api(const float* X, const float* Y, bool on_dev, int B, int T, int accumulation_steps,
                           float* loss_out, float* mask_out, bool mask_on_dev);
    void forward_train_api(const float* X, bool on_dev, int B, int T, float* mask_out, bool mask_on_dev);
    void backward_api(const float* dmask, bool on_dev);
    bool graph_valid = false; int graph_B = 0, graph_T = 0; Tensor graph_f3; float* graph_mask = nullptr;
    int64_t graph_gen = 0;
    void param_arena(float** ptr, int64_t* numel) { *ptr = p_arena; *numel = (int64_t)p_floats; }
    void mark_params_dirty() { affine_dirty = true; }
    void adam_step_api(double lr, double b1, double b2, double eps, double grad_scale);
    void zero_grad_api();
    void adam_state(float* m_host, float* v_host, int64_t numel, int64_t* step, bool set);
    void get_grad(const std::string& key, float* host, int64_t cap_bytes);
    void set_dropout(int mode, unsigned long long seed, const float* masks, int B);
    void grad_arena(float** ptr, int64_t* numel);
    void comm_init(int rank, int world, const void* id128);
    void comm_destroy();
    void allreduce_grads(int wire_dtype);
    void broadcast_params(int root, bool with_optimizer);
    void* comm = nullptr; int comm_rank = 0, comm_world = 1;
    void* wire_buf = nullptr;
private:
    void build_fwd_args(Conv& L, const std::vector<SrcSpec>& srcs, int N, bool batch_as_h, ConvArgs& a);
    Tensor run_conv(Conv& L, const std::vector<SrcSpec>& srcs, int N, const Tensor* out_view, const float* bias,
                    bool batch_as_h);
    template <class F> void for_each_conv(F&& f);
    std::vector<Conv*> conv_layers();
    Tensor run_basenet(BaseNetL& B, const std::vector<SrcSpec>& in, int N, const Tensor* out_view);
    Tensor run_net_window(const Tensor& x, int w_lo, int w_hi);
    Tensor run_lstm(LSTMMod& M, const Tensor& h);
    SrcSpec upsampled(const Tensor& t);
    Tensor run_net(const Tensor& x);
    Tensor net_input(const float* X, const hipMemcpyKind* copy, int B, int T, const float** xd = nullptr);
    void mask_head(const Tensor& f3, int w_lo, int w_hi, HeadDst d);
    void mask_head(const Tensor& f3, int w_lo, int w_hi, float* out);
    void crop_mask_head(const Tensor& f3, int cropsize, HeadDst d);
    void run_dense_crops(float* dense, int count, int cropsize, const HeadDst& d);
    struct StreamStepIO { const float* blk; long long blk_n, blk_pitch; float *y, *v; long long out_pitch, out_off; };
    struct StreamPart {
        StreamState* S; const float* wave; long long n; bool flush; float *y, *v; long long capacity, need;
        long long at; bool flush_done; float *stage_in, *stage_y, *stage_v; StreamStepIO o;
        std::vector<unsigned long long> st;
    };
    struct StreamStepPlan { StreamSeg seg; StreamSchedule p; int new_frames, segments; bool emit; };
    struct StreamCrop { int entry, pass; long long idx; };
    long long stream_check(const StreamState& S, const std::string& who, const float* wave, long long n, bool flush, const float* y,
                           const float* v, bool out_on_dev, long long capacity) const;
    void stream_run(std::vector<StreamPart>& parts, int bs, bool on_dev, bool out_on_dev);
    StreamStepPlan stream_step_plan(StreamState& S, const StreamStepIO& io_, bool final);
    void stream_step_crops(const StreamState& S, const StreamStepPlan& sp, int entry, std::vector<StreamCrop>& list) const;
    void stream_step_commit(StreamState& S, StreamStepIO& io_, const StreamStepPlan& sp);
    void tap(const std::string& name, const Tensor& t);
    bool dry = false;
    const float* dropout_dev = nullptr;
    void plan_and_reserve(int B, int T, size_t extra_bytes);
    void record_begin(int kind, double flops);
    void record_note(double bytes, const char* tag);
    double conv_alg_bytes(const Conv& L, const ConvArgs& a, int N, bool batch_as_h) const;
    void record_end();
};

}
```

vocal-remover_amd/csrc/model.hip:

```cpp
#include "pcm.h"
#include "model.h"

#include <algorithm>
#include <chrono>
#include <cmath>
#include <cstdlib>
#include <cstring>

namespace vr {

static inline int round_up(int v, int m) { return (v + m - 1) / m * m; }

Param* Model::add_param(const std::string& key, std::vector<int64_t> shape, ParamKind kind, bool trainable) {
    params.emplace_back();
    Param* p = &params.back();
    p->key = key;
    p->shape = std::move(shape);
    p->kind = kind;
    p->trainable = trainable;
    p->numel = 1;
    for (auto d : p->shape) p->numel *= (size_t)d;
    p->dev_numel = p->numel;
    if (kind == PK_CONV) {
        p->Cout = (int)p->shape[0];
// ... 255 lines not shown
}

void Model::get_param(const std::string& key, void* host, int64_t cap_bytes) {
    auto it = by_key.find(key);
    VR_CHECK(it != by_key.end(), -2, "unknown parameter key: " + key);
    Param& p = *it->second;
    DeviceGuard dev_guard(device);
    VR_HIP(hipStreamSynchronize(stream));
    if (p.kind == PK_NBT) {
        VR_CHECK(cap_bytes >= 8, -2, "buffer too small");
        *static_cast<int64_t*>(host) = p.nbt;
        return;
    }
    VR_CHECK((size_t)cap_bytes >= p.numel * sizeof(float), -2, "buffer too small for " + key);
    float* dst = static_cast<float*>(host);
    if (p.kind == PK_CONV) {
        std::vector<float> tmp((size_t)p.Cin * p.KK * p.CoutPad);
        VR_HIP(hipMemcpy(tmp.data(), p.dev, tmp.size() * sizeof(float), hipMemcpyDeviceToHost));
        for (int co = 0; co < p.Cout; ++co)
            for (int ci = 0; ci < p.Cin; ++ci)
                for (int k = 0; k < p.KK; ++k)
                    dst[((size_t)co * p.Cin + ci) * p.KK + k] = tmp[((size_t)ci * p.KK + k) * p.CoutPad + co];
    } else if (p.kind == PK_LSTM_IH) {
        std::vector<float> tmp((size_t)p.Cin * p.Cout);
        VR_HIP(hipMemcpy2D(tmp.data(), (size_t)p.Cout * sizeof(float), p.dev + p.co_off, (size_t)p.CoutPad * sizeof(float),
                           (size_t)p.Cout * sizeof(float), (size_t)p.Cin, hipMemcpyDeviceToHost));
        for (int co = 0; co < p.Cout; ++co)
            for (int ci = 0; ci < p.Cin; ++ci) dst[(size_t)co * p.Cin + ci] = tmp[(size_t)ci * p.Cout + co];
    } else {
        VR_HIP(hipMemcpy(dst, p.dev, p.numel * sizeof(float), hipMemcpyDeviceToHost));
    }
}

void Model::need_real_mask(const char* what) const {
    VR_CHECK(!is_complex || complex_train, -2, std::string(what) + ": this handle predicts a complex mask (is_complex=True); only eval-mode inference "
                              "is supported for it, training is not");
}

void Model::need_real_mask_train(const char* what) const {
    VR_CHECK(!(is_complex && training) || complex_train, -2, std::string(what) + " in training mode: this handle predicts a complex mask "
                                            "(is_complex=True); only eval-mode inference is supported for it, training is not");
}

void Model::set_training(bool t) {
    if (training && !t) affine_dirty = true;
    training = t;
}

void Model::fold_eval_affines() {
    if (!affine_dirty) return;
    int maxC = 1;
    for (BN* b : bn_list) maxC = std::max(maxC, std::max(b->C, b->bcast));
    launch_bn_fold_eval(d_fold, (int)bn_list.size(), maxC, 1e-5f, stream);
    refresh_wino(false);
    for (BaseNetL& B : nets_) {
        LSTMMod& M = B.lstm;
        const int G = 4 * M.hid;
        if (!M.bias_sum) VR_HIP(hipMalloc(reinterpret_cast<void**>(&M.bias_sum), (size_t)2 * G * sizeof(float)));
        launch_add(M.b_ih_f->dev, M.b_hh_f->dev, M.bias_sum, G, stream);
        launch_add(M.b_ih_r->dev, M.b_hh_r->dev, M.bias_sum + G, G, stream);
    }
    affine_dirty = false;
}

void Model::set_option(const std::string& name, int value) {
    plan_peak = 0;
    if (name == "train_winograd") train_wino = value != 0;
    else if (name == "serial_exec") serial = value != 0;
    else if (name == "params_dirty") affine_dirty = true;
    else if (name == "mfma_bf16") { mfma_mode = value != 0 ? 1 : default_mfma_mode; affine_dirty = true; }
    else if (name == "mfma_mode") {
        if (value < -1 || value > 3) throw Error(-2, "mfma_mode: 0, 1, 2, 3 or -1 (default)");
        mfma_mode = value < 0 ? default_mfma_mode : value; affine_dirty = true;
    }
    else if (name == "conv_x3d") {
        if (value < -1 || value > 2) throw Error(-2, "conv_x3d: 0, 1, 2 or -1 (default)");
        x3d_mode = value < 0 ? 2 : value;
    }
    else if (name == "conv_x3s") {
        if (value < -1 || value > 1) throw Error(-2, "conv_x3s: 0, 1 or -1 (default)");
        x3s_mode = value < 0 ? x3s_default() : value;
    }
    else if (name == "crop_window") crop_window = value != 0;
    else if (name == "complex_train") {
        if (!is_complex) throw Error(-2, "complex_train: this handle predicts a magnitude mask; the option belongs to complex-mask handles (VR_CREATE_COMPLEX)");
        complex_train = value != 0;
        if (!complex_train && loss_kind != 0) set_loss(0, 0.01);
        graph_valid = false;
    }
    else if (name == "adam_reset") reset_adam_state();
    else if (name == "hip_graph" || name == "conv_x3p" || name == "wgrad_x3h" || name == "conv_x3b") {
        static std::string told;
        if (told.find("|" + name + "|") == std::string::npos) {
            told += "|" + name + "|";
            fprintf(stderr, "libvr_mi355: option '%s' was retired with its kernel (tools/experiments/README.md); ignored\n", name.c_str());
        }
    }
    else throw Error(-2, "unknown option: " + name);
}

void Model::refresh_wino(bool with_dgrad) {
    if (!wino_arena) {
        size_t total = 0;
        for (Conv* L : wino_list) total += (size_t)L->Cin * 16 * L->CoutPad;
        VR_HIP(hipMalloc(reinterpret_cast<void**>(&wino_arena), total * sizeof(float)));
        size_t off = 0;
        for (Conv* L : wino_list) { L->wino = wino_arena + off; off += (size_t)L->Cin * 16 * L->CoutPad; }
    }
    {
        std::vector<WinoWDesc> d;
        for (Conv* L : wino_list) d.push_back(WinoWDesc{L->w->dev, L->wino, L->Cin, L->CoutPad});
        run_wino_batch(wb_fwd, d, false);
    }
    auto cin_pad = [](const Conv* L) { return (L->Cin + 31) / 32 * 32; };
    static const bool x3_on = !(getenv("VR_CONV_X3") && atoi(getenv("VR_CONV_X3")) == 0);
    if (x3_mode() && x3_on) {
        if (!x3_arena) {
            size_t total = 0;
            for (Conv* L : wino_list) total += x3_weights_bytes(L->Cin, 9, L->CoutPad);
            for (Conv* L : x3d_list) total += x3_weights_bytes(L->Cin, L->KS * L->KS, L->CoutPad);
            for (Conv* L : x3s_list) total += x3_weights_bytes(L->Cin, 9, L->CoutPad);
            VR_HIP(hipMalloc(reinterpret_cast<void**>(&x3_arena), total ? total : 16));
            size_t off = 0;
            for (Conv* L : wino_list) { L->x3w = x3_arena + off; off += x3_weights_bytes(L->Cin, 9, L->CoutPad); }
            for (Conv* L : x3d_list) { L->x3w = x3_arena + off; off += x3_weights_bytes(L->Cin, L->KS * L->KS, L->CoutPad); }
            for (Conv* L : x3s_list) { L->x3w = x3_arena + off; off += x3_weights_bytes(L->Cin, 9, L->CoutPad); }
        }
        {
            std::vector<X3WDesc> d;
            for (Conv* L : wino_list) d.push_back(X3WDesc{L->w->dev, L->x3w, L->Cin, 9, L->CoutPad});
            if (mfma_mode == 3) {
                for (Conv* L : x3d_list) d.push_back(X3WDesc{L->w->dev, L->x3w, L->Cin, L->KS * L->KS, L->CoutPad});
                for (Conv* L : x3s_list) d.push_back(X3WDesc{L->w->dev, L->x3w, L->Cin, 9, L->CoutPad});
            }
            run_x3_batch(xb_fwd, d);
        }
        if (with_dgrad) {
            if (!x3t_arena) {
                size_t total = 0;
                for (Conv* L : wino_list) total += x3_weights_bytes(L->Cout, 9, cin_pad(L));
                for (Conv* L : x3d_list) total += x3_weights_bytes(L->Cout, L->KS * L->KS, cin_pad(L));
                VR_HIP(hipMalloc(reinterpret_cast<void**>(&x3t_arena), total ? total : 16));
                size_t off = 0;
                for (Conv* L : wino_list) { x3t_of[L->w] = x3t_arena + off; off += x3_weights_bytes(L->Cout, 9, cin_pad(L)); }
                for (Conv* L : x3d_list) { x3dt_of[L->w] = x3t_arena + off; off += x3_weights_bytes(L->Cout, L->KS * L->KS, cin_pad(L)); }
            }
            std::vector<X3WDesc> d;
            for (Conv* L : wino_list) {
                auto it = wt_of.find(L->w);
                if (it != wt_of.end()) d.push_back(X3WDesc{it->second, x3t_of[L->w], L->Cout, 9, cin_pad(L)});
            }
            if (mfma_mode == 3)
                for (Conv* L : x3d_list) {
                    auto it = wt_of.find(L->w);
                    if (it != wt_of.end()) d.push_back(X3WDesc{it->second, x3dt_of[L->w], L->Cout, L->KS * L->KS, cin_pad(L)});
                }
            run_x3_batch(xb_bwd, d);
        }
    }
    if (mfma_mode == 2 && !x3_on) {
        auto fwd6 = [](const Conv* L) { return L->CoutPad % 64 == 0; };
        auto bwd6 = [&](const Conv* L) { return cin_pad(L) % 64 == 0; };
        if (!wino6_arena) {
            size_t total = 0;
            for (Conv* L : wino_list) if (fwd6(L)) total += wino_weights6_bytes(L->Cin, L->CoutPad);
            VR_HIP(hipMalloc(reinterpret_cast<void**>(&wino6_arena), total ? total : 16));
// ... 203 lines not shown
int64_t Model::get_tap(const std::string& name, float* host, int64_t cap_floats, int64_t* shape4) {
    DeviceGuard dev_guard(device);
    auto it = taps.find(name);
    VR_CHECK(it != taps.end(), -2, "no such tap: " + name);
    const Tensor& t = it->second;
    const int64_t n = (int64_t)t.N * t.C * t.H * t.W;
    if (shape4) { shape4[0] = t.N; shape4[1] = t.C; shape4[2] = t.H; shape4[3] = t.W; }
    if (!host) return n;
    VR_CHECK(cap_floats >= n, -2, "tap buffer too small");
    float* tmp = nullptr;
    VR_HIP(hipMalloc(&tmp, n * sizeof(float)));
    launch_materialize(t, tmp, stream);
    VR_HIP(hipStreamSynchronize(stream));
    VR_HIP(hipMemcpy(host, tmp, n * sizeof(float), hipMemcpyDeviceToHost));
    VR_HIP(hipFree(tmp));
    return n;
}

ConvSrc make_src(const Tensor& t, bool up, int bcastH) {
    ConvSrc s{};
    s.p = t.p; s.aff0 = t.aff0; s.aff1 = t.aff1 ? t.aff1 : t.aff0;
    s.sN = t.sN; s.sC = t.sC; s.sH = t.sH;
    s.C = t.C; s.H = t.H; s.W = t.W;
    s.hsplit = t.hsplit; s.slope = t.slope; s.up = up ? 1 : 0; s.post = t.post; s.zins = 0;
    s.rh = (t.H > 0) ? (float)(t.H - 1) / (float)(2 * t.H - 1) : 0.f;
    s.rw = (t.W > 0) ? (float)(t.W - 1) / (float)(2 * t.W - 1) : 0.f;
    if (bcastH) { s.sH = 0; s.H = bcastH; }
    return s;
}

void Model::build_fwd_args(Conv& L, const std::vector<SrcSpec>& srcs, int N, bool batch_as_h, ConvArgs& a) {
    VR_CHECK(!srcs.empty() && srcs.size() <= 3, -2, "conv " + L.name + ": 1..3 sources");
    a = ConvArgs{};
    a.nsrc = (int)srcs.size();
    int Hin = -1, Win = -1, ctot = 0;
    for (int i = 0; i < a.nsrc; ++i) {
        const SrcSpec& sp = srcs[i];
        a.src[i] = make_src(sp.t, sp.up, sp.bcastH);
        const int vh = sp.up ? 2 * sp.t.H : (sp.bcastH ? sp.bcastH : sp.t.H);
        const int vw = sp.up ? 2 * sp.t.W : sp.t.W;
        if (sp.plain) {
            ConvSrc& c = a.src[i];
            c = ConvSrc{};
            c.p = sp.plain; c.C = sp.t.C; c.H = vh; c.W = vw;
            c.sH = vw; c.sC = (long long)vh * vw; c.sN = c.sC * sp.t.C;
            c.hsplit = 1 << 30; c.slope = 1.f;
        }
        if (Hin < 0) { Hin = vh; Win = vw; }
        VR_CHECK(vh == Hin && vw == Win, -5, "h1_shape[3] must be greater than h2_shape[3] (decoder skip/upsample size mismatch in " + L.name + ")");
        ctot += sp.t.C;
    }
    VR_CHECK(ctot == L.Cin, -2, "conv " + L.name + ": channel count mismatch");
    {
        const ConvSrc* u = nullptr;
        for (int i = 0; i < a.nsrc; ++i) {
            if (!a.src[i].up) continue;
            if (u) VR_CHECK(u->H == a.src[i].H && u->W == a.src[i].W && u->sH == a.src[i].sH, -2,
                            "conv " + L.name + ": upsampled sources must share H, W and row stride");
            u = &a.src[i];
        }
    }
    a.c1 = a.nsrc >= 2 ? srcs[0].t.C : L.Cin;
    a.c2 = a.nsrc >= 3 ? srcs[0].t.C + srcs[1].t.C : L.Cin;
    a.Cin = L.Cin;
    a.w = L.w->dev;
    a.Cout = L.Cout; a.CoutPad = L.CoutPad;
    a.d1 = a.d2 = 1 << 30;
    int Nk = N;
    if (batch_as_h) {
        VR_CHECK(L.KS == 1 && Hin == 1, -2, "batch-as-rows view needs a 1x1 conv on H=1 input");
        for (int i = 0; i < a.nsrc; ++i) {
            VR_CHECK(!a.src[i].post && !a.src[i].up, -2, "batch-as-rows: unsupported source flags");
            a.src[i].sH = a.src[i].sN; a.src[i].sN = 0; a.src[i].H = N;
        }
        Hin = N; Nk = 1;
    }
    a.N = Nk; a.Hin = Hin; a.Win = Win;
    a.Hout = (Hin + 2 * L.pad_h - L.dh * (L.KS - 1) - 1) / L.stride + 1;
    a.Wout = (Win + 2 * L.pad_w - L.dw * (L.KS - 1) - 1) / L.stride + 1;
    a.pad_h = L.pad_h; a.pad_w = L.pad_w;
}

Tensor Model::run_conv(Conv& L, const std::vector<SrcSpec>& srcs_in, int N, const Tensor* out_view, const float* bias,
                       bool batch_as_h) {
    std::vector<SrcSpec> srcs = srcs_in;
    static const bool mat_enabled = !getenv("VR_NO_TRAIN_MAT");
    if (training && mat_enabled) {
        for (SrcSpec& sp : srcs) {
            const Tensor& t = sp.t;
            if (!(t.aff0 || t.aff1 || t.post || t.slope != 1.f || sp.up || sp.bcastH)) continue;
            const int vh = sp.up ? 2 * t.H : (sp.bcastH ? sp.bcastH : t.H), vw = sp.up ? 2 * t.W : t.W;
            float* buf = ws.allocf((size_t)t.N * t.C * vh * vw);
            if (!dry) {
                if (sp.up) launch_upsample2x(t, buf, stream);
                else {
                    Tensor v = t;
                    if (sp.bcastH) { v.H = sp.bcastH; v.sH = 0; }
                    launch_materialize(v, buf, stream);
                }
            }
            sp.plain = buf;
        }
    }
    ConvArgs a;
    build_fwd_args(L, srcs, N, batch_as_h, a);
    if (!training) {
        bool any_up = false;
        for (const SrcSpec& sp : srcs) any_up = any_up || sp.up;
        if (any_up) {
            ConvArgs probe = a;
            probe.x3w = x3_mode() ? L.x3w : nullptr;
            probe.bf16 = mfma_mode;
            X3Tile xt;
            if (!x3_pick(probe, ConvShape{L.KS, L.stride, L.dh, L.dw}, &xt)) {
                for (SrcSpec& sp : srcs) {
                    if (!sp.up) continue;
                    const Tensor& t = sp.t;
                    Tensor u;
                    u.N = t.N; u.C = t.C; u.H = 2 * t.H; u.W = 2 * t.W;
                    u.sH = u.W; u.sC = (long long)u.H * u.W; u.sN = u.sC * u.C; u.slope = 1.f;
                    u.p = ws.allocf((size_t)u.N * u.C * u.H * u.W);
                    if (!dry) launch_upsample2x(t, u.p, stream);
                    sp = SrcSpec{u};
                }
                build_fwd_args(L, srcs, N, batch_as_h, a);
            }
        }
    }
    a.bias = bias;
    const bool fuse_epi = !training && L.bn != nullptr;
    if (fuse_epi) { a.epi = L.bn->affine; a.epi_slope = L.slope; }
    a.wino = (training && !train_wino) ? nullptr : L.wino;
    a.wino6 = (a.wino && mfma_mode == 2) ? L.wino6 : nullptr;
    a.x3w = (x3_mode() && !(training && !train_wino)) ? L.x3w : nullptr;
    if (!x3d_mode && a.Win == 16) a.x3w = nullptr;
    if (L.stride == 2 && (training || !x3s_mode)) a.x3w = nullptr;
    a.bf16 = mfma_mode;
    int wcols = a.Wout;
    if (conv_w_hi > 0 && !training && mfma_mode == 3 && !batch_as_h && !conv_sink) {
        X3Tile xt;
        int tth;
        const ConvShape cs{L.KS, L.stride, L.dh, L.dw};
        if (!thin16_pick(a, cs, &tth) && x3_pick(a, cs, &xt)) {
            a.w_lo = conv_w_lo; a.w_hi = conv_w_hi;
            wcols = std::min(a.Wout, (conv_w_hi + 31) / 32 * 32) - conv_w_lo / 32 * 32;
        }
    }
    Tensor o;
    if (batch_as_h) {
        o.N = N; o.C = L.Cout; o.H = 1; o.W = a.Wout;
        if (out_view) { o.p = out_view->p; o.g = out_view->g; o.sN = out_view->sN; o.sC = out_view->sC; o.sH = out_view->sH; }
        else {
            o.p = ws.allocf((size_t)N * L.Cout * a.Wout); o.sN = (long long)L.Cout * a.Wout; o.sC = a.Wout; o.sH = a.Wout;
            if (taping()) o.g = galloc((size_t)N * L.Cout * a.Wout, false);
        }
        a.dst[0] = ConvDst{o.p, 0, o.sC, o.sN, 0};
    } else {
        o.N = N; o.C = L.Cout; o.H = a.Hout; o.W = a.Wout;
        if (out_view) {
            VR_CHECK(out_view->H == a.Hout && out_view->W == a.Wout && out_view->C == L.Cout, -2, "conv " + L.name + ": output view shape mismatch");
            o.p = out_view->p; o.g = out_view->g; o.sN = out_view->sN; o.sC = out_view->sC; o.sH = out_view->sH;
        } else {
            o.p = ws.allocf((size_t)N * L.Cout * a.Hout * a.Wout);
            o.sH = a.Wout; o.sC = (long long)a.Hout * a.Wout; o.sN = o.sC * L.Cout;
            if (taping()) o.g = galloc((size_t)N * L.Cout * a.Hout * a.Wout, true);
        }
        a.dst[0] = ConvDst{o.p, o.sN, o.sC, o.sH, 0};
    }
    const ConvShape shp{L.KS, L.stride, L.dh, L.dw};
    const bool stats = training && L.bn;
    size_t npt = 0;
    if (stats) {
        npt = conv_part_count(a, shp);
        a.part = ws.allocf(npt * L.Cout * 2);
    }
    if (!dry && conv_sink) {
        PendingConv pc{};
        pc.a = a; pc.shp = shp;
        pc.flops = 2.0 * N * (double)a.Hout * a.Wout * (double)L.Cout * L.Cin * L.KS * L.KS;
        pc.bytes = conv_alg_bytes(L, a, N, batch_as_h);
        pc.stats = stats; pc.bn = L.bn;
        if (stats) {
            BNFinalizeArgs& f = pc.fin;
            f.part = a.part; f.nparts = (int)npt; f.pstride = L.Cout * 2;
            f.count = (double)N * a.Hout * a.Wout;
            f.w = L.bn->w->dev; f.b = L.bn->b->dev; f.rm = L.bn->rm->dev; f.rv = L.bn->rv->dev;
            f.affine = L.bn->affine; f.save_mean = L.bn->save_mean; f.save_invstd = L.bn->save_invstd;
            f.C = L.Cout; f.eps = 1e-5f; f.momentum = 0.1f; f.broadcast = 0;
        }
        conv_sink->push_back(pc);
    } else if (!dry) {
        const double flops = 2.0 * N * (double)(batch_as_h ? 1 : a.Hout) * wcols * (double)L.Cout * L.Cin * L.KS * L.KS;
        record_begin(0, flops);
        if (profiling) {
            char tag[160];
            snprintf(tag, sizeof tag, "%s k%d s%d d%d ci%d co%d %dx%dx%d", L.name.c_str(), L.KS, L.stride, L.dh, L.Cin,
                     L.Cout, a.N, a.Hout, a.Wout);
            double bytes = conv_alg_bytes(L, a, N, batch_as_h);
            if (wcols < a.Wout) {
                const double fi = std::min(1.0, (wcols + 2.0) / a.Win), fo = (double)wcols / a.Wout;
                bytes = 4.0 * ((double)a.N * L.Cin * a.Hin * a.Win * fi + (double)N * L.Cout * a.Hout * a.Wout * fo +
                               (double)L.Cin * L.KS * L.KS * L.Cout);
                snprintf(tag + strlen(tag), sizeof tag - strlen(tag), " cols %d-%d", a.w_lo / 32 * 32, a.w_lo / 32 * 32 + wcols);
            }
            record_note(bytes, tag);
        }
        launch_conv(a, shp, stream);
        record_end();
        if (stats) {
            BNFinalizeArgs f{};
            f.part = a.part; f.nparts = (int)npt; f.pstride = L.Cout * 2;
            f.count = (double)N * (batch_as_h ? 1 : a.Hout) * a.Wout;
            f.w = L.bn->w->dev; f.b = L.bn->b->dev; f.rm = L.bn->rm->dev; f.rv = L.bn->rv->dev;
            f.affine = L.bn->affine; f.save_mean = L.bn->save_mean; f.save_invstd = L.bn->save_invstd;
            f.C = L.Cout; f.eps = 1e-5f; f.momentum = 0.1f; f.broadcast = 0;
            launch_bn_finalize(f, stream);
            L.bn->nbt->nbt += 1;
        }
    }
    if (L.bn && !fuse_epi) { o.aff0 = L.bn->affine; o.slope = L.slope; } else { o.aff0 = nullptr; o.slope = 1.f; }
    if (taping()) {
        TapeRec r;
        r.kind = TK_CONV; r.L = &L; r.srcs = srcs; r.out = o; r.N = N; r.batch_as_h = batch_as_h; r.bias = bias;
        tape.push_back(std::move(r));
    }
    return o;
}

Tensor Model::run_lstm(LSTMMod& M, const Tensor& h) {
    const int N = h.N, nb = h.H, nf = h.W;
    VR_CHECK(nb == M.nin, -2, "LSTM input size does not match the number of bins at dec2");
    float* z = ws.allocf((size_t)N * nb * nf);
    const int nblk = launch_squeeze_conv(h, M.squeeze.w->dev, z, nullptr, true, stream);
    float* part = training ? ws.allocf((size_t)nblk * 2) : nullptr;
    if (!dry) {
        launch_squeeze_conv(h, M.squeeze.w->dev, z, part, false, stream, training ? nullptr : M.squeeze.bn->affine);
        if (training) {
            BN* b = M.squeeze.bn;
            BNFinalizeArgs f{};
            f.part = part; f.nparts = nblk; f.pstride = 2; f.count = (double)N * nb * nf;
            f.w = b->w->dev; f.b = b->b->dev; f.rm = b->rm->dev; f.rv = b->rv->dev;
            f.affine = b->affine; f.save_mean = b->save_mean; f.save_invstd = b->save_invstd;
            f.C = 1; f.eps = 1e-5f; f.momentum = 0.1f; f.broadcast = b->bcast;
            launch_bn_finalize(f, stream);
            b->nbt->nbt += 1;
        }
    }
    Tensor zt;
    zt.p = z; zt.N = N; zt.C = nb; zt.H = 1; zt.W = nf;
    zt.sN = (long long)nb * nf; zt.sC = nf; zt.sH = nf;
    if (training) { zt.aff0 = M.squeeze.bn->affine; zt.slope = 0.f; }
    else zt.slope = 1.f;
    if (taping()) {
        zt.g = galloc((size_t)N * nb * nf, false);
        TapeRec r;
        r.kind = TK_SQUEEZE; r.M = &M; r.srcs = {SrcSpec{h}}; r.N = N;
        r.out = zt;
        r.out.C = 1; r.out.H = nb; r.out.sC = (long long)nb * nf; r.out.sH = nf;
        tape.push_back(std::move(r));
    }
    const int G = 4 * M.hid;
    float* bias = ws.allocf((size_t)2 * G);
    if (!training && M.bias_sum) bias = M.bias_sum;
    else if (!dry) {
        launch_add(M.b_ih_f->dev, M.b_hh_f->dev, bias, G, stream);
        launch_add(M.b_ih_r->dev, M.b_hh_r->dev, bias + G, G, stream);
    }
    Tensor gx = run_conv(M.proj, {SrcSpec{zt}}, N, nullptr, bias, true);
    float* hc = ws.allocf((size_t)N * 2 * M.hid * nf);
    float* save = taping() ? ws.allocf((size_t)N * 2 * nf * 5 * M.hid) : nullptr;
    if (!dry) launch_bilstm_train(gx.p, M.whh_f->dev, M.whh_r->dev, hc, save, N, nf, M.hid, stream);
    Tensor ht;
    ht.p = hc; ht.N = N; ht.C = 2 * M.hid; ht.H = 1; ht.W = nf;
    ht.sN = (long long)2 * M.hid * nf; ht.sC = nf; ht.sH = nf; ht.slope = 1.f;
    if (taping()) {
        ht.g = galloc((size_t)N * 2 * M.hid * nf, false);
        TapeRec r;
        r.kind = TK_LSTM; r.M = &M; r.N = N; r.out = ht; r.aux = gx; r.save = save;
        tape.push_back(std::move(r));
    }
    Tensor lin = run_conv(M.dense, {SrcSpec{ht}}, N, nullptr, M.dense_b->dev, true);
    if (taping()) tape.back().bias_param = M.dense_b;
    float* act = training ? ws.allocf((size_t)N * nb * nf) : lin.p;
    if (!dry && training) launch_rows_affine_relu(lin.p, act, M.dense.bn->affine, N, nb, nf, stream);
    Tensor o;
    o.p = act; o.g = lin.g; o.N = N; o.C = 1; o.H = nb; o.W = nf;
    o.sN = (long long)nb * nf; o.sC = (long long)nb * nf; o.sH = nf; o.slope = 1.f;
    return o;
}

Model::SrcSpec Model::upsampled(const Tensor& t) {
    if (training) {
        SrcSpec s{t};
        s.up = true;
        return s;
    }
    static const bool fuse_on = !(getenv("VR_X3_FUSE_UP") && atoi(getenv("VR_X3_FUSE_UP")) == 0);
    static const bool x3_on = !(getenv("VR_CONV_X3") && atoi(getenv("VR_CONV_X3")) == 0);
    if (fuse_on && x3_on && x3_mode() && 4LL * t.H * t.W >= 65536 && 2 * t.W >= 32 && !t.aff0 && !t.aff1 && !t.post && t.slope == 1.f) {
        SrcSpec s{t};
        s.up = true;
        return s;
    }
    Tensor u;
    u.N = t.N; u.C = t.C; u.H = 2 * t.H; u.W = 2 * t.W;
    u.sH = u.W; u.sC = (long long)u.H * u.W; u.sN = u.sC * u.C; u.slope = 1.f;
    u.p = ws.allocf((size_t)u.N * u.C * u.H * u.W);
    if (!dry) launch_upsample2x(t, u.p, stream);
    return SrcSpec{u};
}

Tensor Model::run_basenet(BaseNetL& B, const std::vector<SrcSpec>& in, int N, const Tensor* out_view) {
    const std::string& p = B.prefix;
    Tensor e[5];
    e[0] = run_conv(B.enc1, in, N, nullptr, nullptr, false);
    tap(p + ".e1", e[0]);
    for (int i = 0; i < 4; ++i) {
        Tensor t = run_conv(B.enc_a[i], {SrcSpec{e[i]}}, N, nullptr, nullptr, false);
        e[i + 1] = run_conv(B.enc_b[i], {SrcSpec{t}}, N, nullptr, nullptr, false);
        tap(p + ".e" + std::to_string(i + 2), e[i + 1]);
    }
    const Tensor& x5 = e[4];
    const int C8 = 8 * B.c;
    float* pooled = ws.allocf((size_t)N * C8 * x5.W);
    if (!dry) launch_avgpool_h(x5, pooled, stream);
    Tensor pt;
    pt.p = pooled; pt.N = N; pt.C = C8; pt.H = 1; pt.W = x5.W;
    pt.sN = (long long)C8 * x5.W; pt.sC = x5.W; pt.sH = x5.W; pt.slope = 1.f;
    if (taping()) {
        pt.g = galloc((size_t)N * C8 * x5.W, false);
        TapeRec r;
        r.kind = TK_AVGPOOL; r.srcs = {SrcSpec{x5}}; r.out = pt; r.N = N;
        tape.push_back(std::move(r));
    }
    Tensor f1 = run_conv(B.aspp_pool, {SrcSpec{pt}}, N, nullptr, nullptr, true);
    Tensor cat4;
    cat4.N = N; cat4.C = 4 * C8; cat4.H = x5.H; cat4.W = x5.W;
    cat4.sH = x5.W; cat4.sC = (long long)x5.H * x5.W; cat4.sN = cat4.sC * cat4.C;
    cat4.p = ws.allocf((size_t)N * cat4.C * x5.H * x5.W);
    if (taping()) cat4.g = galloc((size_t)N * cat4.C * x5.H * x5.W, false);
    if (training) { cat4.aff0 = B.aspp_aff; cat4.slope = 0.f; }
    Conv* branch[4] = {&B.aspp_c2, &B.aspp_d[0], &B.aspp_d[1], &B.aspp_d[2]};
    Tensor x5b = x5;
    {
        static const bool mat_enabled = !getenv("VR_NO_TRAIN_MAT");
        if (training && mat_enabled && (x5.aff0 || x5.aff1 || x5.post || x5.slope != 1.f)) {
            float* buf = ws.allocf((size_t)N * C8 * x5.H * x5.W);
            if (!dry) launch_materialize(x5, buf, stream);
            x5b.p = buf; x5b.aff0 = x5b.aff1 = nullptr; x5b.post = nullptr; x5b.slope = 1.f; x5b.hsplit = 1 << 30;
            x5b.sH = x5.W; x5b.sC = (long long)x5.H * x5.W; x5b.sN = x5b.sC * C8;
        }
    }
    static const bool aspp_fork = !getenv("VR_NO_ASPP_FORK");
    std::vector<PendingConv> pend;
    const bool group = !dry && mfma_mode == 3 && x3d_mode == 2 && !(training && !train_wino);
    const bool afk = aspp_fork && !serial && !training && !dry && !profiling && side_stream != nullptr && !band_fork_active && !group;
    hipStream_t aspp_main = stream;
    if (afk) {
        hipEvent_t ef = ev_fork;
        VR_HIP(hipEventRecord(ef, aspp_main));
        VR_HIP(hipStreamWaitEvent(side_stream, ef, 0));
    }
    for (int j = 0; j < 4; ++j) {
        Tensor v = cat4;
        v.C = C8;
        v.p = dry ? cat4.p : cat4.p + (long long)j * C8 * cat4.sC;
        if (taping() && !dry) v.g = cat4.g + (long long)j * C8 * cat4.sC;
        if (afk) stream = (j & 1) ? side_stream : aspp_main;
        if (group) conv_sink = &pend;
        try { run_conv(*branch[j], {SrcSpec{x5b}}, N, &v, nullptr, false); } catch (...) { stream = aspp_main; conv_sink = nullptr; throw; }
        conv_sink = nullptr;
    }
    if (group) {
        VR_CHECK(pend.size() == 4, -3, "ASPP: four branch convs expected");
        ConvArgs c4[4];
        ConvShape s4[4];
        double flops = 0.0, bytes = 0.0;
        for (int j = 0; j < 4; ++j) { c4[j] = pend[j].a; s4[j] = pend[j].shp; flops += pend[j].flops; bytes += pend[j].bytes; }
        if (x3d_aspp_eligible(c4, s4)) {
            record_begin(0, flops);
            if (profiling) {
                char tag[160];
                snprintf(tag, sizeof tag, "%s.aspp.conv2-5 k1+3x(k3 d4/8/12) ci%d co%d %dx%dx%d", p.c_str(), C8, C8, N, x5.H, x5.W);
                record_note(bytes - 3.0 * 4.0 * (double)N * C8 * x5.H * x5.W, tag);
            }
            x3d_launch_aspp(c4, stream);
            record_end();
        } else {
            for (int j = 0; j < 4; ++j) {
                record_begin(0, pend[j].flops);
                if (profiling) record_note(pend[j].bytes, branch[j]->name.c_str());
                launch_conv(c4[j], s4[j], stream);
                record_end();
            }
        }
        for (int j = 0; j < 4; ++j)
            if (pend[j].stats) {
                launch_bn_finalize(pend[j].fin, stream);
                pend[j].bn->nbt->nbt += 1;
            }
    }
    if (afk) {
        stream = aspp_main;
        hipEvent_t ej = ev_join;
        VR_HIP(hipEventRecord(ej, side_stream));
        VR_HIP(hipStreamWaitEvent(aspp_main, ej, 0));
    }
    SrcSpec s1{f1};
    s1.bcastH = x5.H;
    Tensor h = run_conv(B.aspp_bott, {s1, SrcSpec{cat4}}, N, nullptr, nullptr, false);
    if (training && dropout_dev) {
        int idx = (int)(&B - nets_);
        h.post = dropout_dev + (size_t)idx * N * 8 * nout;
        if (taping()) tape.back().out.post = h.post;
    }
    tap(p + ".aspp", h);
    for (int i = 0; i < 3; ++i) {
        SrcSpec up = upsampled(h);
        h = run_conv(B.dec[i], {up, SrcSpec{e[3 - i]}}, N, nullptr, nullptr, false);
        tap(p + ".dec" + std::to_string(4 - i), h);
    }
    static const bool lstm_fork = !getenv("VR_NO_LSTM_FORK");
    const bool fk = lstm_fork && !serial && !training && !dry && !profiling && side_stream != nullptr && !band_fork_active;
    SrcSpec uh;
    hipEvent_t lstm_join = nullptr;
    if (fk) {
        hipStream_t ms = stream;
        hipEvent_t ef = ev_fork;
        VR_HIP(hipEventRecord(ef, ms));
        VR_HIP(hipStreamWaitEvent(side_stream, ef, 0));
        stream = side_stream;
        try { uh = upsampled(h); } catch (...) { stream = ms; throw; }
        lstm_join = ev_join;
        VR_HIP(hipEventRecord(lstm_join, side_stream));
        stream = ms;
    }
    Tensor l = run_lstm(B.lstm, h);
    tap(p + ".lstm", l);
    if (fk) VR_HIP(hipStreamWaitEvent(stream, lstm_join, 0));
    else uh = upsampled(h);
    SrcSpec ul = upsampled(l);
    const bool win = &B == &nets_[4] && net_w_hi > 0;
    if (win) { conv_w_lo = net_w_lo; conv_w_hi = net_w_hi; }
    Tensor o;
    try { o = run_conv(B.dec[3], {uh, ul, SrcSpec{e[0]}}, N, out_view, nullptr, false); } catch (...) { conv_w_lo = conv_w_hi = 0; throw; }
    conv_w_lo = conv_w_hi = 0;
    tap(p + ".dec1", o);
    return o;
}

Tensor Model::run_net(const Tensor& x) {
    const int B = x.N, T = x.W;
    const int bandw = max_bin / 2;
    Tensor xl = x; xl.H = bandw;
    Tensor xh = x; xh.H = bandw; xh.p = dry ? x.p : x.p + (long long)bandw * x.sH;
    auto make_aux = [&](int C) {
        Tensor t;
        t.N = B; t.C = C; t.H = max_bin; t.W = T;
        t.sH = T; t.sC = (long long)max_bin * T; t.sN = t.sC * C;
        t.p = ws.allocf((size_t)B * C * max_bin * T);
        if (taping()) t.g = galloc((size_t)B * C * max_bin * T, false);
        t.slope = training ? 0.f : 1.f;
        return t;
    };
    Tensor aux1 = make_aux(nout / 4), aux2 = make_aux(nout / 2);
    auto half = [&](const Tensor& a, int which) {
        Tensor v = a; v.H = bandw;
        if (which && !dry) { v.p = a.p + (long long)bandw * a.sH; if (a.g) v.g = a.g + (long long)bandw * a.sH; }
        return v;
    };
    Tensor v;
    static const bool train_fork = !getenv("VR_NO_TRAIN_FORK");
    static const bool band_fork = !getenv("VR_NO_BAND_FORK");
    const bool fork = band_fork && !serial && !dry && (!training || train_fork) && !profiling && side_stream != nullptr;
    hipStream_t main_stream = stream;
    if (fork) {
        hipEvent_t ef = ev_fork;
        VR_HIP(hipEventRecord(ef, main_stream));
        VR_HIP(hipStreamWaitEvent(side_stream, ef, 0));
        band_fork_active = true;
    }
    Tensor l1r = run_basenet(nets_[0], {SrcSpec{xl}}, B, nullptr);
    v = half(aux1, 0);
    Tensor l1 = run_conv(tail1, {SrcSpec{l1r}}, B, &v, nullptr, false);
    Tensor l2r = run_basenet(nets_[2], {SrcSpec{xl}, SrcSpec{l1}}, B, nullptr);
    v = half(aux2, 0);
    Tensor l2 = run_conv(tail2, {SrcSpec{l2r}}, B, &v, nullptr, false);
    if (fork) stream = side_stream;
    const size_t tape_hi0 = tape.size();
    v = half(aux1, 1);
    Tensor h1 = run_basenet(nets_[1], {SrcSpec{xh}}, B, &v);
    v = half(aux2, 1);
    Tensor h2 = run_basenet(nets_[3], {SrcSpec{xh}, SrcSpec{h1}}, B, &v);
    for (size_t i = tape_hi0; i < tape.size(); ++i) tape[i].chain = 1;
    if (fork) {
        hipEvent_t ej = ev_join;
        VR_HIP(hipEventRecord(ej, side_stream));
        stream = main_stream;
        VR_HIP(hipStreamWaitEvent(main_stream, ej, 0));
        band_fork_active = false;
    }
    tap("l1", l1); tap("h1", h1);
    tap("l2", l2); tap("h2", h2);
    aux1.aff0 = l1.aff0; aux1.aff1 = h1.aff0; aux1.hsplit = bandw;
    aux2.aff0 = l2.aff0; aux2.aff1 = h2.aff0; aux2.hsplit = bandw;
    Tensor xf = x; xf.H = max_bin;
    Tensor f3 = run_basenet(nets_[4], {SrcSpec{xf}, SrcSpec{aux1}, SrcSpec{aux2}}, B, nullptr);
    return f3;
}

Tensor Model::run_net_window(const Tensor& x, int w_lo, int w_hi) {
    if (!(crop_window && !training && mfma_mode == 3 && !record_taps && w_hi > 0 && w_lo > 0)) return run_net(x);
    net_w_lo = w_lo; net_w_hi = w_hi;
    Tensor f3;
    try { f3 = run_net(x); } catch (...) { net_w_lo = net_w_hi = 0; throw; }
    net_w_lo = net_w_hi = 0;
    return f3;
}

void Model::plan_and_reserve(int B, int T, size_t extra_bytes) {
    graph_valid = false;
    if (plan_B == B && plan_T == T && plan_training == training && plan_peak > 0) {
        ensure_ws(plan_peak + extra_bytes + 4096);
        ws.reset();
        return;
    }
    Arena saved = ws;
    ws.dry = true; ws.base = nullptr; ws.off = 0; ws.peak = 0;
    dry = true;
    Tensor x;
    x.p = reinterpret_cast<float*>(uintptr_t(256));
    x.N = B; x.C = nin; x.H = max_bin; x.W = T; x.sH = T; x.sC = (long long)output_bin * T; x.sN = nin * x.sC;
    try { run_net(x); } catch (...) { dry = false; ws = saved; throw; }
    dry = false;
    const size_t need = ws.peak + extra_bytes + 4096;
    plan_B = B; plan_T = T; plan_training = training; plan_peak = ws.peak;
    ws = saved;
    ensure_ws(need);
    ws.reset();
}

static void check_T(int T, int offset, int mode) {
    VR_CHECK(T > 0 && T % 16 == 0, -5, "h1_shape[3] must be greater than h2_shape[3] (frames must be a multiple of 16)");
    if (mode != 0) VR_CHECK(T - 2 * offset > 0, -6, "assert mask.size()[3] > 0 (frames must exceed 2*offset)");
}

template <bool CPLX>
__global__ void mul_crop_kernel(const float* __restrict__ x, float* __restrict__ m, int T, int Wm, int off, long long total) {
    const long long gid = (long long)blockIdx.x * blockDim.x + threadIdx.x;
    if (gid >= total) return;
    const int w = (int)(gid % Wm);
    const long long row = gid / Wm;
    if constexpr (CPLX) {
        const float2 a = reinterpret_cast<const float2*>(x)[row * T + off + w];
        float2* mc = reinterpret_cast<float2*>(m) + gid;
        const float2 b = *mc;
        *mc = make_float2(a.x * b.x - a.y * b.y, a.x * b.y + a.y * b.x);
    } else {
        m[gid] *= x[row * T + off + w];
    }
}

void launch_mul_crop(const float* x, float* m, bool cplx, long long rows, int T, int Wm, int off, hipStream_t st) {
    const long long total = rows * Wm;
    if (cplx) VR_LAUNCH((mul_crop_kernel<true>), dim3((unsigned)((total + 255) / 256)), dim3(256), 0, st, x, m, T, Wm, off, total);
    else VR_LAUNCH((mul_crop_kernel<false>), dim3((unsigned)((total + 255) / 256)), dim3(256), 0, st, x, m, T, Wm, off, total);
    VR_HIP(hipGetLastError());
}

Tensor Model::net_input(const float* X, const hipMemcpyKind* copy, int B, int T, const float** xd) {
// ... 1108 lines not shown
```

vocal-remover_amd/csrc/vr_common.h:

```cpp
#pragma once
#include <hip/hip_runtime.h>
#include <atomic>
#include <cstdint>
#include <cstdio>
#include <stdexcept>
#include <string>
#include <vector>

namespace vr {

struct Error : std::runtime_error {
    int code;
    Error(int c, const std::string& m) : std::runtime_error(m), code(c) {}
};

#define VR_HIP(expr)                                                                              \
    do {                                                                                          \
        hipError_t _e = (expr);                                                                   \
        if (_e != hipSuccess)                                                                     \
            throw ::vr::Error(-3, std::string(#expr) + ": " + hipGetErrorString(_e));             \
    } while (0)

#define VR_CHECK(cond, code, msg)                                                                 \
    do {                                                                                          \
// ... 21 lines not shown
    DeviceGuard& operator=(const DeviceGuard&) = delete;
};

struct LaunchProfiler;
extern thread_local LaunchProfiler* g_launch_prof;
void prof_note(double flops, double bytes, bool strong = false, const char* tag = nullptr);
void prof_note_update(double bytes, const char* tag);
void prof_note_clear();
LaunchProfiler* prof_create();
void prof_destroy(LaunchProfiler* p);
bool prof_owned_by_this_thread(const LaunchProfiler* p);
void prof_abandon(LaunchProfiler* p);
void prof_collect(LaunchProfiler* p, double* conv_ms, double* conv_flops, double* conv_bytes, int* conv_launches, std::string* report,
                  bool dump);
void prof_before(const void* fn, const char* label, hipStream_t st);
void prof_after(hipStream_t st);
void prof_memset_async(void* p, int value, size_t bytes, hipStream_t st);

#define VR_LAUNCH(kern, grid, block, lds, st, ...)                                                                     \
    do {                                                                                                               \
        if (::vr::g_launch_prof) ::vr::prof_before(reinterpret_cast<const void*>(kern), #kern, st);                    \
        hipLaunchKernelGGL(kern, grid, block, lds, st, __VA_ARGS__);                                                   \
        if (::vr::g_launch_prof) ::vr::prof_after(st);                                                                 \
    } while (0)

struct Tensor {
    float* p = nullptr;
    int N = 0, C = 0, H = 0, W = 0;
    long long sN = 0, sC = 0, sH = 0;
    const float* aff0 = nullptr;
    const float* aff1 = nullptr;
    int hsplit = 1 << 30;
    float slope = 1.f;
    const float* post = nullptr;
    float* g = nullptr;
};

struct ConvSrc {
    const float* p;
    const float* aff0;
    const float* aff1;
    long long sN, sC, sH;
    int C, H, W;
    int hsplit;
    float slope;
    int up;
    float rh, rw;
    const float* post;
    int zins;
};

struct ConvDst {
    float* p;
    long long sN, sC, sH;
    int accumulate;
    int wshift;
};

struct ConvArgs {
    ConvSrc src[3];
    int nsrc, c1, c2;
    int Cin;
    const float* w;
    const float* wino;
    const void* wino6;
    const void* x3w;
    const float* bias;
    int Cout, CoutPad;
    ConvDst dst[3];
    int d1, d2;
    float* part;
    const float* epi;
    float epi_slope;
    int N, Hout, Wout, Hin, Win;
    int pad_h, pad_w;
    int tiles_w, tiles_h, npt, nct;
    int dbg;
    int bf16;
    long long s2_cls_stride;
    int s2_H, s2_W;
    int tapmask;
    int w_lo, w_hi;
    int wt0;
};

struct ConvShape {
    int KS, stride, dil_h, dil_w;
};

struct WgradArgs {
    ConvArgs in;
    const float* dz;
    long long zN, zC, zH;
    int Cout, CoutPad;
    float* part;
    long long part_stride;
    int P, tiles_w, tiles_h, npt, nchunks, nct;
    int dma;
    int bf16;
    int allow_wino;
};
double launch_wgrad(const WgradArgs& a, const ConvShape& s, float* grad_out, int accumulate, hipStream_t st);
struct WgReduceDesc { const float* part; long long stride; float* out; long long n; int P; int accumulate; long long blk0; };
void wgrad_defer_to(std::vector<WgReduceDesc>* sink);
int wgrad_reduce_vec(const WgReduceDesc* host_descs, int n);
void launch_wgrad_reduce_batched(const WgReduceDesc* d_descs, int n, long long total_blocks, int vec, hipStream_t st);
size_t wgrad_scratch_floats(const WgradArgs& a, const ConvShape& s);
void launch_wgrad_reduce(const float* part, long long stride, int P, float* out, long long n, int accumulate, hipStream_t st);

double launch_conv(const ConvArgs& a, const ConvShape& s, hipStream_t st);
size_t conv_part_count(const ConvArgs& a, const ConvShape& s);
void conv_fill_tiling(ConvArgs& a, const ConvShape& s);
bool conv_dma_eligible(const ConvArgs& a, const ConvShape& s);

}
```

Baseline: 188,500 spectrogram-frames/sec.

## Fuse following 1x1 conv and LSTM squeeze into conv_x3h epilogue

Adds a second-stage tail to the conv_x3h kernel. The epilogue can now apply a 1x1 conv with BN and activation (the low-band tail1/tail2 layers) or the LSTM squeeze conv directly on the accumulators, using cross-half lane permutes and weights staged in LDS. This removes a separate kernel launch and a full write and re-read of the intermediate activation for those layers. The cost is extra LDS and registers in the conv kernel, which may lower occupancy, plus stricter eligibility rules with a fallback to the unfused path.

```diff
diff --git a/vocal-remover_amd/csrc/conv_mfma.hip b/vocal-remover_amd/csrc/conv_mfma.hip
--- a/vocal-remover_amd/csrc/conv_mfma.hip
+++ b/vocal-remover_amd/csrc/conv_mfma.hip
@@ -353,6 +353,12 @@
         VR_CHECK(a.bf16 == 3 && a.nsrc >= 1 && a.nsrc <= 3 && a.w_lo >= 0 && a.w_lo < a.w_hi && !a.part && x3_pick(a, s, &x3t), -2,
                  "conv column window: only conv_x3h (mfma_mode 3, eval) takes one");
     }
+    if (a.tail) {
+        X3Tile x3t;
+        int th;
+        VR_CHECK(a.bf16 == 3 && a.nsrc >= 1 && a.nsrc <= 3 && !thin16_pick(a, s, &th) && x3_pick(a, s, &x3t), -2,
+                 "conv with a second stage in its epilogue: only conv_x3h (mfma_mode 3, eval) takes one");
+    }
     for (int i = 0; i < a.nsrc && i < 3; ++i) {
         const ConvSrc& c = a.src[i];
         VR_CHECK(!(c.up && c.aff1 && c.aff1 != c.aff0 && c.hsplit < c.H), -2, "conv: an upsampled source cannot carry a row-split affine (hsplit)");
diff --git a/vocal-remover_amd/csrc/conv_x3h.hip b/vocal-remover_amd/csrc/conv_x3h.hip
--- a/vocal-remover_amd/csrc/conv_x3h.hip
+++ b/vocal-remover_amd/csrc/conv_x3h.hip
@@ -2,6 +2,7 @@
 #include <type_traits>
 
 #include "conv_epilogue.h"
+#include "conv_x3h_tail.h"
 #include "conv_stage.h"
 #include "kernels.h"
 #include "lds_dma.h"
@@ -9,7 +10,7 @@
 
 namespace vr {
 
-template <int MT, int TH, bool UP = true>
+template <int MT, int TH, bool UP = true, int TAIL = 0>
 struct X3hCfg {
     static constexpr int TW = 32, CK = 8, KK = 9;
     static constexpr int TH_in = TH + 2, PW = TW + 2;
@@ -26,7 +27,9 @@
     static constexpr int L_BYTES = UP ? CK * LSLOT * 4 : 0;
     static constexpr int E_OFF = L_OFF + L_BYTES;
     static constexpr int M_OFF = E_OFF + 4 * MT * 4;
-    static constexpr int LDS_BYTES = M_OFF + 16;
+    static constexpr int T_OFF = M_OFF + 16;
+    static constexpr int T_BYTES = TAIL == 1 ? (32 * 16 + 32) * 4 : (TAIL == 2 ? (MT + 4) * 4 : 0);
+    static constexpr int LDS_BYTES = T_OFF + T_BYTES;
     static constexpr int OCC = (MT == 32 && TH == 8) ? 3 : 2;
     static constexpr int NXL = 8 * NPASS, NWMIN = (NWP / 64) / 4;
     static constexpr int NG = 14;
@@ -42,9 +45,9 @@
     VR_HIP(hipMemcpyToSymbol(HIP_SYMBOL(g_x3h_trace), zeros, sizeof zeros));
 }
 
-template <int MT, int TH, bool UP, bool HI, bool TRACE = false>
+template <int MT, int TH, bool UP, bool HI, bool TRACE = false, int TAIL = 0>
 __global__ __launch_bounds__(256, (X3hCfg<MT, TH>::OCC + (HI ? 1 : 0))) void conv_x3h_kernel(const ConvArgs a) {
-    using Cfg = X3hCfg<MT, TH, UP>;
+    using Cfg = X3hCfg<MT, TH, UP, TAIL>;
     constexpr int TW = Cfg::TW, KK = Cfg::KK, PW = Cfg::PW, NSLOT = Cfg::NSLOT, NPASS = Cfg::NPASS, WM = Cfg::WM, WN = Cfg::WN,
                   PLANE = Cfg::PLANE, NWP = Cfg::NWP, NWPASS = Cfg::NWPASS;
     extern __shared__ __attribute__((aligned(16))) char smem_x3h[];
@@ -282,6 +285,24 @@
         ecv[2] = x3h_load(re, ecc * 8 + 4);
         ecv[3] = x3h_load(rw, ec * 4);
     }
+    float tcv[3] = {0.f, 0.f, 0.f};
+    if constexpr (TAIL != 0) {
+        i32x4 r2 = make_rsrc(a.t_w, 0x7FFFFFF0u), r3 = make_rsrc(a.t_epi, 0x7FFFFFF0u);
+        settle_rsrc(r2);
+        settle_rsrc(r3);
+        constexpr int OOB = (int)0x80000000u;
+        if constexpr (TAIL == 1) {
+#pragma unroll
+            for (int q = 0; q < 2; ++q) {
+                const int c = (tid + 256 * q) >> 4, j = tid & 15;
+                tcv[q] = x3h_load(r2, (c < a.Cout && j < a.t_Cout) ? (c * a.t_CoutPad + j) * 4 : OOB);
+            }
+            tcv[2] = x3h_load(r3, tid < 2 * a.t_Cout ? tid * 4 : OOB);
+        } else {
+            tcv[0] = x3h_load(r2, tid < a.Cout ? tid * 4 : OOB);
+            tcv[1] = x3h_load(r3, tid < 2 ? tid * 4 : OOB);
+        }
+    }
     auto follow = [&](int e, bool first) {
         const int need = 140 - (e < 14 ? 14 : e);
         shlo = (first || need < shlo) ? need : shlo;
@@ -320,6 +341,18 @@
         E[MT + tid] = a.epi ? ecv[1] : 1.f;
         E[2 * MT + tid] = a.epi ? ecv[2] : 0.f;
         E[3 * MT + tid] = ecv[3];
+    }
+    if constexpr (TAIL != 0) {
+        asm volatile("; landed %0 %1 %2" : "+v"(tcv[0]), "+v"(tcv[1]), "+v"(tcv[2]));
+        float* T = reinterpret_cast<float*>(smem_x3h + Cfg::T_OFF);
+        if constexpr (TAIL == 1) {
+            T[tid] = tcv[0];
+            T[256 + tid] = tcv[1];
+            if (tid < 32) T[512 + tid] = tcv[2];
+        } else {
+            if (tid < MT) T[tid] = tcv[0];
+            if (tid < 2) T[MT + tid] = tcv[1];
+        }
     }
     post_max(P0{});
     if (any_up) stage_lowres(P0{});
@@ -426,12 +459,18 @@
                     for (int j = 0; j < 4; ++j) acc[mi][ni][rq * 4 + j] = (acc[mi][ni][rq * 4 + j] * fo) * wi[j];
             }
     }
-    {
+    if constexpr (TAIL != 1) {
         int hon[WN], won[WN];
 #pragma unroll
         for (int ni = 0; ni < WN; ++ni) { hon[ni] = h0 + wave * WN + ni; won[ni] = w0 + l31; }
         epi_store<MT, WM, WN>(VR_EPI_ARGS(a), acc, reinterpret_cast<const float*>(smem_x3h + Cfg::E_OFF), n, co0, khalf,
                               h0 + TH <= a.Hout && w0 + TW <= a.Wout, hon, won);
+    }
+    if constexpr (TAIL != 0) {
+        x3h_second_stage<MT, WM, WN, TAIL>(acc, reinterpret_cast<const float*>(smem_x3h + Cfg::E_OFF), reinterpret_cast<const float*>(smem_x3h + Cfg::T_OFF),
+                                   a.epi ? a.epi_slope : 1.f, a.t_slope, a.t_Cout, a.t_p, a.t_sN, a.t_sC, a.t_sH, n, h0 + wave * WN, w0 + l31,
+                                   a.Hout, a.Wout, khalf, lane);
+        return;
     }
     if (a.part) {
         __syncthreads();
@@ -564,7 +603,35 @@
     else x3h_launch_up<MT, TH, false, false>(a, st);
 }
 
+template <int MT, int TH, bool UP, int TAIL>
+static void x3h_launch_tail(const ConvArgs& a, hipStream_t st) {
+    using Cfg = X3hCfg<MT, TH, UP, TAIL>;
+    auto kern = conv_x3h_kernel<MT, TH, UP, (TH == 8 && !UP), false, TAIL>;
+    static std::atomic<unsigned long long> attr_done{0};
+    ensure_lds_attr(attr_done, reinterpret_cast<const void*>(kern), Cfg::LDS_BYTES);
+    VR_LAUNCH(kern, dim3((a.npt + 7) / 8 * 8), dim3(256), Cfg::LDS_BYTES, st, a);
+    VR_HIP(hipGetLastError());
+}
+
+bool x3h_tail_ok(const ConvArgs& a, const X3Tile& t) {
+    if (a.tail != 1 && a.tail != 2) return false;
+    if (a.bf16 != 3 || a.nct != 1 || a.Cout > t.MT || a.part || a.w_hi != 0 || !a.t_w || !a.t_epi || !a.t_p) return false;
+    const bool up = (a.src[0].up | (a.nsrc > 1 ? a.src[1].up : 0) | (a.nsrc > 2 ? a.src[2].up : 0)) != 0;
+    if (a.tail == 1) return t.MT == 32 && t.TH == 16 && up && a.t_Cout >= 1 && a.t_Cout <= 16 && a.t_CoutPad >= a.t_Cout;
+    if (a.d1 < a.Cout || !a.dst[0].p || a.dst[0].accumulate || a.dst[0].wshift) return false;
+    return t.TH == 8 && (t.MT == 64 || (t.MT == 32 && !up));
+}
+
 void x3h_launch_conv(const ConvArgs& a, const X3Tile& t, hipStream_t st) {
+    if (a.tail) {
+        VR_CHECK(x3h_tail_ok(a, t), -2, "conv_x3h: no kernel for this launch with a second stage (x3h_tail_ok)");
+        const bool up = (a.src[0].up | a.src[1].up | a.src[2].up) != 0;
+        if (a.tail == 1) x3h_launch_tail<32, 16, true, 1>(a, st);
+        else if (t.MT == 32) x3h_launch_tail<32, 8, false, 2>(a, st);
+        else if (up) x3h_launch_tail<64, 8, true, 2>(a, st);
+        else x3h_launch_tail<64, 8, false, 2>(a, st);
+        return;
+    }
     if (t.MT == 64) x3h_launch<64, 8>(a, st);
     else if (t.TH == 16) x3h_launch<32, 16>(a, st);
     else x3h_launch<32, 8>(a, st);
diff --git a/vocal-remover_amd/csrc/conv_x3h_tail.h b/vocal-remover_amd/csrc/conv_x3h_tail.h
--- /dev/null
+++ b/vocal-remover_amd/csrc/conv_x3h_tail.h
@@ -0,0 +1,171 @@
+#pragma once
+#include "conv_epilogue.h"
+#include "x3h_common.h"
+
+namespace vr {
+
+typedef float vr_epi_f4 __attribute__((ext_vector_type(4)));
+
+template <int K>
+__device__ __forceinline__ void x3h_other_half(const float (&v)[K], float (&o)[K], int lane) {
+    const int addr = (lane ^ 32) * 4;
+#pragma unroll
+    for (int i = 0; i < K; ++i)
+        asm volatile("ds_bpermute_b32 %0, %1, %2" : "=v"(o[i]) : "v"(addr), "v"(v[i]));
+    asm volatile("s_waitcnt lgkmcnt(0)" ::: "memory");
+#pragma unroll
+    for (int i = 0; i < K; ++i) asm volatile("" : "+v"(o[i]));
+}
+
+template <int WN, int J>
+__device__ __forceinline__ void x3h_tail_mix(f32x16 (&acc)[1][WN], const float* T, float tslope, int tCout, float* tp, long long tsN,
+                                             long long tsC, long long tsH, int n, int hrow0, int wcol, int Hout, int Wout, int khalf, int lane) {
+    constexpr int H = J / 2, CB = 32 / H;
+    constexpr int NP = 2;
+    static_assert(WN % NP == 0, "pixel groups");
+    float s2[H], b2[H];
+#pragma unroll
+    for (int jj = 0; jj < H; ++jj) {
+        s2[jj] = T[512 + 2 * (khalf * H + jj)];
+        b2[jj] = T[512 + 2 * (khalf * H + jj) + 1];
+    }
+    asm volatile("s_waitcnt lgkmcnt(0)" ::: "memory");
+#pragma unroll
+    for (int jj = 0; jj < H; ++jj) asm volatile("" : "+v"(s2[jj]), "+v"(b2[jj]));
+    float* const q0 = tp + (long long)n * tsN + (long long)(khalf * H) * tsC + wcol;
+    const unsigned wl = (unsigned)(size_t)T + (unsigned)(khalf * H * 4);
+    static_for<WN / NP>([&](auto pass) {
+        constexpr int n0 = decltype(pass)::value * NP;
+        float mine[16 * NP], oth[16 * NP];
+#pragma unroll
+        for (int r = 0; r < 16; ++r)
+#pragma unroll
+            for (int ni = 0; ni < NP; ++ni) mine[r * NP + ni] = acc[0][n0 + ni][r];
+        x3h_other_half<16 * NP>(mine, oth, lane);
+        float y[H][NP];
+#pragma unroll
+        for (int jj = 0; jj < H; ++jj)
+#pragma unroll
+            for (int ni = 0; ni < NP; ++ni) y[jj][ni] = 0.f;
+        static_for<32 / CB>([&](auto batch) {
+            constexpr int cb = decltype(batch)::value;
+            vr_epi_f4 q[CB][H / 4];
+#pragma unroll
+            for (int i = 0; i < CB; ++i)
+#pragma unroll
+                for (int j4 = 0; j4 < H / 4; ++j4)
+                    asm volatile("ds_read_b128 %0, %1 offset:%2" : "=v"(q[i][j4]) : "v"(wl), "n"(((cb * CB + i) * 16 + 4 * j4) * 4));
+            asm volatile("s_waitcnt lgkmcnt(0)" ::: "memory");
+            float w[CB][H];
+#pragma unroll
+            for (int i = 0; i < CB; ++i)
+#pragma unroll
+                for (int j4 = 0; j4 < H / 4; ++j4) {
+                    asm volatile("" : "+v"(q[i][j4]));
+#pragma unroll
+                    for (int e = 0; e < 4; ++e) w[i][4 * j4 + e] = q[i][j4][e];
+                }
+            static_for<CB>([&](auto ch) {
+                constexpr int i = decltype(ch)::value, c = cb * CB + i;
+                constexpr int r = (c >> 3) * 4 + (c & 3);
+                constexpr bool upper = ((c >> 2) & 1) != 0;
+#pragma unroll
+                for (int ni = 0; ni < NP; ++ni) {
+                    float av = (upper == (khalf != 0)) ? mine[r * NP + ni] : oth[r * NP + ni];
+                    asm volatile("" : "+v"(av));
+#pragma unroll
+                    for (int jj = 0; jj < H; ++jj) y[jj][ni] = fmaf(w[i][jj], av, y[jj][ni]);
+                }
+            });
+#pragma unroll
+            for (int jj = 0; jj < H; ++jj)
+#pragma unroll
+                for (int ni = 0; ni < NP; ++ni) asm volatile("" : "+v"(y[jj][ni]));
+        });
+#pragma unroll
+        for (int jj = 0; jj < H; ++jj)
+#pragma unroll
+            for (int ni = 0; ni < NP; ++ni) {
+                const float v = act_apply(fmaf(y[jj][ni], s2[jj], b2[jj]), tslope);
+                const int ho = hrow0 + n0 + ni;
+                if (khalf * H + jj < tCout && ho < Hout && wcol < Wout) q0[(long long)jj * tsC + (long long)ho * tsH] = v;
+            }
+    });
+}
+
+template <int MT, int WM, int WN, int TAIL>
+__device__ __forceinline__ void x3h_second_stage(f32x16 (&acc)[WM][WN], const float* E, const float* T, float eslope, float tslope, int tCout, float* tp,
+                                         long long tsN, long long tsC, long long tsH, int n, int hrow0, int wcol, int Hout, int Wout, int khalf,
+                                         int lane) {
+    static_assert(TAIL == 2 || (MT == 32 && WM == 1), "the stage tail takes one 32-cout block");
+#pragma unroll
+    for (int mi = 0; mi < WM; ++mi)
+#pragma unroll
+        for (int rq = 0; rq < 4; ++rq) {
+            const int cb = mi * 32 + 8 * rq + 4 * khalf;
+            const vr_epi_f4 b4 = *reinterpret_cast<const vr_epi_f4*>(E + cb), s4 = *reinterpret_cast<const vr_epi_f4*>(E + MT + cb),
+                            h4 = *reinterpret_cast<const vr_epi_f4*>(E + 2 * MT + cb);
+            float eb[4], esc[4], esh[4];
+#pragma unroll
+            for (int j = 0; j < 4; ++j) { eb[j] = b4[j]; esc[j] = s4[j]; esh[j] = h4[j]; }
+            asm volatile("s_waitcnt lgkmcnt(0)" ::: "memory");
+#pragma unroll
+            for (int j = 0; j < 4; ++j) asm volatile("" : "+v"(eb[j]), "+v"(esc[j]), "+v"(esh[j]));
+#pragma unroll
+            for (int ni = 0; ni < WN; ++ni)
+#pragma unroll
+                for (int j = 0; j < 4; ++j) {
+                    float v = acc[mi][ni][rq * 4 + j];
+                    if constexpr (TAIL == 1) v += eb[j];
+                    acc[mi][ni][rq * 4 + j] = act_apply(fmaf(v, esc[j], esh[j]), eslope);
+                }
+        }
+    if constexpr (TAIL == 1) {
+        if (tCout <= 8) x3h_tail_mix<WN, 8>(acc, T, tslope, tCout, tp, tsN, tsC, tsH, n, hrow0, wcol, Hout, Wout, khalf, lane);
+        else x3h_tail_mix<WN, 16>(acc, T, tslope, tCout, tp, tsN, tsC, tsH, n, hrow0, wcol, Hout, Wout, khalf, lane);
+    } else {
+        float wv[WM * 16];
+#pragma unroll
+        for (int mi = 0; mi < WM; ++mi)
+#pragma unroll
+            for (int rq = 0; rq < 4; ++rq) {
+                const vr_epi_f4 q = *reinterpret_cast<const vr_epi_f4*>(T + mi * 32 + 8 * rq + 4 * khalf);
+#pragma unroll
+                for (int j = 0; j < 4; ++j) wv[mi * 16 + rq * 4 + j] = q[j];
+            }
+        float s2 = T[MT], b2 = T[MT + 1];
+        asm volatile("s_waitcnt lgkmcnt(0)" ::: "memory");
+#pragma unroll
+        for (int i = 0; i < WM * 16; ++i) asm volatile("" : "+v"(wv[i]));
+        asm volatile("" : "+v"(s2), "+v"(b2));
+        float z[WN];
+#pragma unroll
+        for (int ni = 0; ni < WN; ++ni) z[ni] = 0.f;
+#pragma unroll
+        for (int sg = 0; sg < 8 * WM; ++sg) {
+            const int mi = sg >> 3, rq = (sg & 7) >> 1;
+            const bool owner = (khalf != 0) == ((sg & 1) != 0);
+            if (sg > 0) {
+                float zo[WN];
+                x3h_other_half<WN>(z, zo, lane);
+#pragma unroll
+                for (int ni = 0; ni < WN; ++ni) z[ni] = owner ? zo[ni] : z[ni];
+            }
+#pragma unroll
+            for (int ni = 0; ni < WN; ++ni) {
+                float t = z[ni];
+#pragma unroll
+                for (int j = 0; j < 4; ++j) t = fmaf(wv[mi * 16 + rq * 4 + j], acc[mi][ni][rq * 4 + j], t);
+                z[ni] = owner ? t : z[ni];
+            }
+        }
+        float* const q0 = tp + (long long)n * tsN + wcol;
+#pragma unroll
+        for (int ni = 0; ni < WN; ++ni) {
+            const float v = fmaxf(fmaf(z[ni], s2, b2), 0.f);
+            if (khalf && hrow0 + ni < Hout && wcol < Wout) q0[(long long)(hrow0 + ni) * tsH] = v;
+        }
+    }
+}
+
+}
diff --git a/vocal-remover_amd/csrc/debug.hip b/vocal-remover_amd/csrc/debug.hip
--- a/vocal-remover_amd/csrc/debug.hip
+++ b/vocal-remover_amd/csrc/debug.hip
@@ -351,6 +351,106 @@
     }
 }
 
+void Model::debug_conv_tail(const int64_t* dims, int ndims, const float* fp, int nfp, const float* const* in, int nin, float* const* out,
+                            int nout) {
+    const std::string who = "vr_debug_kernel(conv_tail): ";
+    VR_CHECK(ndims >= 12 && nfp >= 2 && nout >= 2, -2, who + "too few arguments");
+    const int nsrc = (int)dims[0], N = (int)dims[1], Cout = (int)dims[2], kind = (int)dims[3], Cout2 = (int)dims[4];
+    const X3Tile tile{(int)dims[5], (int)dims[6]};
+    VR_CHECK(nsrc >= 1 && nsrc <= 3 && N >= 1 && Cout >= 1 && (kind == 1 || kind == 2) && Cout2 >= 1 && (kind == 1 || Cout2 == 1), -2,
+             who + "1..3 sources, kind 1 or 2");
+    VR_CHECK((tile.MT == 32 || tile.MT == 64) && (tile.TH == 8 || (tile.TH == 16 && tile.MT == 32)), -2, who + "tilings: <32,8>, <32,16>, <64,8>");
+    VR_CHECK(mfma_mode == 3, -2, who + "conv_x3h runs in mfma_mode 3");
+    VR_CHECK(ndims >= 12 + 9 * nsrc && nin >= 5 + nsrc && in[0] && in[1] && in[2] && in[3] && in[4] && out[0], -2, who + "too few arguments");
+    ConvArgs a{};
+    a.nsrc = nsrc; a.N = N; a.Cout = Cout; a.CoutPad = (Cout + 31) / 32 * 32;
+    VR_CHECK(a.CoutPad % tile.MT == 0, -2, who + "the cout tile does not divide the padded couts");
+    a.d1 = a.d2 = 1 << 30;
+    a.bf16 = 3;
+    a.pad_h = a.pad_w = 1;
+    std::vector<std::unique_ptr<DevBuf>> keep;
+    auto upload = [&](const float* host, size_t n) { keep.emplace_back(new DevBuf(host, n)); return keep.back()->p; };
+    int Cin = 0;
+    const ConvSrc* ups = nullptr;
+    for (int i = 0; i < nsrc; ++i) {
+        const int64_t* d = dims + 12 + 9 * i;
+        Tensor t;
+        t.N = N; t.C = (int)d[0]; t.H = (int)d[1]; t.W = (int)d[2];
+        const bool up = d[3] != 0;
+        const size_t floats = (size_t)d[4];
+        t.sN = d[6]; t.sC = d[7]; t.sH = d[8];
+        VR_CHECK(in[5 + i] && view_fits(d[5], t.sN, t.sC, t.sH, N, t.C, t.H, t.W, floats), -2, who + "a source view leaves its buffer");
+        t.p = upload(in[5 + i], floats) + d[5];
+        t.slope = 1.f;
+        a.src[i] = make_src(t, up, 0);
+        const int vh = up ? 2 * t.H : t.H, vw = up ? 2 * t.W : t.W;
+        if (i == 0) { a.Hin = vh; a.Win = vw; }
+        VR_CHECK(vh == a.Hin && vw == a.Win, -2, who + "the sources must share the input size");
+        if (up && ups) VR_CHECK(ups->H == t.H && ups->W == t.W && ups->sH == t.sH, -2, who + "upsampled sources must share H, W and row stride");
+        if (up) ups = &a.src[i];
+        Cin += t.C;
+        if (i == 0) a.c1 = Cin;
+        if (i <= 1) a.c2 = Cin;
+    }
+    a.Cin = Cin;
+    a.Hout = a.Hin; a.Wout = a.Win;
+    const int H = a.Hout, W = a.Wout;
+    std::vector<float> wk((size_t)Cin * 9 * a.CoutPad, 0.f);
+    for (int co = 0; co < Cout; ++co)
+        for (int ci = 0; ci < Cin; ++ci)
+            for (int k = 0; k < 9; ++k) wk[((size_t)ci * 9 + k) * a.CoutPad + co] = in[0][((size_t)co * Cin + ci) * 9 + k];
+    DevBuf dwk(wk.data(), wk.size());
+    a.w = dwk.p;
+    a.epi = upload(in[1], (size_t)Cout * 2); a.epi_slope = fp[0];
+    DebugWeightForms wf;
+    debug_weight_forms(dwk.p, Cin, 3, 1, 1, 1, a.CoutPad, a.Win, true, a, wf);
+    {
+        X3Tile any;
+        VR_CHECK(a.x3w && x3_pick(a, ConvShape{3, 1, 1, 1}, &any), -2, who + "conv_x3h does not take this launch");
+    }
+    const int CoutPad2 = (Cout2 + 31) / 32 * 32;
+    std::vector<float> w2((size_t)Cout * (kind == 1 ? CoutPad2 : 1), 0.f);
+    for (int j = 0; j < Cout2; ++j)
+        for (int c = 0; c < Cout; ++c) w2[kind == 1 ? (size_t)c * CoutPad2 + j : (size_t)c] = in[2][(size_t)j * Cout + c];
+    DevBuf dw2(w2.data(), w2.size());
+    const float* epi2 = upload(in[3], (size_t)Cout2 * 2);
+    const size_t yfloats = (size_t)dims[7];
+    const long long yoff = kind == 1 ? dims[8] : 0, ysN = kind == 1 ? dims[9] : (long long)H * W, ysC = kind == 1 ? dims[10] : 0,
+                    ysH = kind == 1 ? dims[11] : W;
+    VR_CHECK(view_fits(yoff, ysN, kind == 1 ? ysC : 1, ysH, N, kind == 1 ? Cout2 : 1, H, W, yfloats), -2, who + "the view of y leaves its buffer");
+    GuardedBuf y(in[4], yfloats);
+    DevBuf prod((size_t)N * Cout * H * W);
+    a.dst[0] = ConvDst{prod.p, (long long)Cout * H * W, (long long)H * W, W, 0, 0};
+    x3_fill_tiling(a, tile);
+    if (fuse_tail) {
+        a.tail = kind; a.t_Cout = Cout2; a.t_CoutPad = kind == 1 ? CoutPad2 : 1; a.t_w = dw2.p; a.t_epi = epi2; a.t_slope = fp[1];
+        a.t_p = y.p() + yoff; a.t_sN = ysN; a.t_sC = ysC; a.t_sH = ysH;
+        VR_CHECK(x3h_tail_ok(a, tile), -2, who + "conv_x3h has no kernel for this launch with a second stage (x3h_tail_ok)");
+        x3h_launch_conv(a, tile, stream);
+    } else {
+        x3h_launch_conv(a, tile, stream);
+        const Tensor pt = dense(prod.p, N, Cout, H, W);
+        if (kind == 1) {
+            ConvArgs b{};
+            b.nsrc = 1; b.N = N; b.Cin = Cout; b.c1 = b.c2 = Cout; b.Cout = Cout2; b.CoutPad = CoutPad2;
+            b.d1 = b.d2 = 1 << 30;
+            b.bf16 = 3;
+            b.src[0] = make_src(pt, false, 0);
+            b.Hin = b.Hout = H; b.Win = b.Wout = W;
+            b.w = dw2.p;
+            b.epi = epi2; b.epi_slope = fp[1];
+            b.dst[0] = ConvDst{y.p() + yoff, ysN, ysC, ysH, 0, 0};
+            launch_conv(b, ConvShape{1, 1, 1, 1}, stream);
+        } else {
+            launch_squeeze_conv(pt, dw2.p, y.p(), nullptr, false, stream, epi2);
+        }
+    }
+    VR_HIP(hipStreamSynchronize(stream));
+    VR_CHECK(y.intact(), -3, who + "a launch stored outside y's buffer");
+    y.download(out[0]);
+    prod.download(out[1]);
+}
+
 void Model::debug_wgrad_launch(const int64_t* dims, int ndims, const float* fp, int nfp, const float* const* in, int nin, float* const* out,
                                int nout) {
     const std::string who = "vr_debug_kernel(wgrad_launch): ";
@@ -610,6 +710,7 @@
         return;
     }
     if (name == "conv_launch") { debug_conv_launch(dims, ndims, fp, nfp, in, nin, out, nout); return; }
+    if (name == "conv_tail") { debug_conv_tail(dims, ndims, fp, nfp, in, nin, out, nout); return; }
     if (name == "wgrad_launch") { debug_wgrad_launch(dims, ndims, fp, nfp, in, nin, out, nout); return; }
     if (name == "wgrad_reduce") { debug_wgrad_reduce(dims, ndims, in, nin, out, nout); return; }
     if (name == "dgrad_launch") { debug_dgrad_launch(dims, ndims, in, nin, out, nout); return; }
diff --git a/vocal-remover_amd/csrc/kernels.h b/vocal-remover_amd/csrc/kernels.h
--- a/vocal-remover_amd/csrc/kernels.h
+++ b/vocal-remover_amd/csrc/kernels.h
@@ -62,6 +62,7 @@
 void launch_x3_weights(const float* w, void* o, int Cin, int KK, int CoutPad, hipStream_t st);
 void launch_x3_weights_batched(const X3WDesc* d_descs, int n, long long max_elems, hipStream_t st);
 void x3h_launch_conv(const ConvArgs& a, const X3Tile& t, hipStream_t st);
+bool x3h_tail_ok(const ConvArgs& a, const X3Tile& t);
 void x3h_trace_read(long long* host, int n);
 void x3h_trace_clear();
 void launch_x3h_weights(const float* w, void* o, int Cin, int KK, int CoutPad, hipStream_t st);
diff --git a/vocal-remover_amd/csrc/model.h b/vocal-remover_amd/csrc/model.h
--- a/vocal-remover_amd/csrc/model.h
+++ b/vocal-remover_amd/csrc/model.h
@@ -203,6 +203,8 @@
 
     void debug_conv_launch(const int64_t* dims, int ndims, const float* fp, int nfp, const float* const* in, int nin, float* const* out,
                            int nout);
+    void debug_conv_tail(const int64_t* dims, int ndims, const float* fp, int nfp, const float* const* in, int nin, float* const* out,
+                         int nout);
     void debug_wgrad_launch(const int64_t* dims, int ndims, const float* fp, int nfp, const float* const* in, int nin, float* const* out,
                             int nout);
     void debug_wgrad_reduce(const int64_t* dims, int ndims, const float* const* in, int nin, float* const* out, int nout);
@@ -263,6 +265,7 @@
     int default_mfma_mode = 3;
     bool serial = false;
     bool crop_window = true;
+    bool fuse_tail = true;
     int net_w_lo = 0, net_w_hi = 0;
     void set_option(const std::string& name, int value);
     void reset_adam_state();
@@ -431,13 +434,14 @@
     void* wire_buf = nullptr;
 private:
     void build_fwd_args(Conv& L, const std::vector<SrcSpec>& srcs, int N, bool batch_as_h, ConvArgs& a);
+    struct FusedTail { int kind = 0; Conv* L = nullptr; LSTMMod* M = nullptr; Tensor out; bool done = false; };
     Tensor run_conv(Conv& L, const std::vector<SrcSpec>& srcs, int N, const Tensor* out_view, const float* bias,
-                    bool batch_as_h);
+                    bool batch_as_h, FusedTail* tail = nullptr);
     template <class F> void for_each_conv(F&& f);
     std::vector<Conv*> conv_layers();
-    Tensor run_basenet(BaseNetL& B, const std::vector<SrcSpec>& in, int N, const Tensor* out_view);
+    Tensor run_basenet(BaseNetL& B, const std::vector<SrcSpec>& in, int N, const Tensor* out_view, FusedTail* tail = nullptr);
     Tensor run_net_window(const Tensor& x, int w_lo, int w_hi);
-    Tensor run_lstm(LSTMMod& M, const Tensor& h);
+    Tensor run_lstm(LSTMMod& M, const Tensor& h, float* z, bool squeezed);
     SrcSpec upsampled(const Tensor& t);
     Tensor run_net(const Tensor& x);
     Tensor net_input(const float* X, const hipMemcpyKind* copy, int B, int T, const float** xd = nullptr);
diff --git a/vocal-remover_amd/csrc/model.hip b/vocal-remover_amd/csrc/model.hip
--- a/vocal-remover_amd/csrc/model.hip
+++ b/vocal-remover_amd/csrc/model.hip
@@ -361,6 +361,7 @@
         x3s_mode = value < 0 ? x3s_default() : value;
     }
     else if (name == "crop_window") crop_window = value != 0;
+    else if (name == "fuse_tail") fuse_tail = value != 0;
     else if (name == "complex_train") {
         if (!is_complex) throw Error(-2, "complex_train: this handle predicts a magnitude mask; the option belongs to complex-mask handles (VR_CREATE_COMPLEX)");
         complex_train = value != 0;
@@ -730,7 +731,7 @@
 }
 
 Tensor Model::run_conv(Conv& L, const std::vector<SrcSpec>& srcs_in, int N, const Tensor* out_view, const float* bias,
-                       bool batch_as_h) {
+                       bool batch_as_h, FusedTail* tail) {
     std::vector<SrcSpec> srcs = srcs_in;
     static const bool mat_enabled = !getenv("VR_NO_TRAIN_MAT");
     if (training && mat_enabled) {
@@ -822,6 +823,37 @@
         npt = conv_part_count(a, shp);
         a.part = ws.allocf(npt * L.Cout * 2);
     }
+    const char* fused_tag = "";
+    if (tail && !dry && fuse_tail && !training && mfma_mode == 3 && !record_taps && !conv_sink && !batch_as_h && fuse_epi && a.w_hi == 0) {
+        X3Tile xt;
+        int tth;
+        if (!thin16_pick(a, shp, &tth) && x3_pick(a, shp, &xt)) {
+            ConvArgs b = a;
+            x3_fill_tiling(b, xt);
+            b.tail = tail->kind;
+            b.t_p = tail->out.p;
+            if (tail->kind == 1) {
+                const Conv& L2 = *tail->L;
+                VR_CHECK(L2.KS == 1 && L2.Cin == L.Cout && L2.bn && tail->out.C == L2.Cout && tail->out.H == a.Hout && tail->out.W == a.Wout, -3,
+                         "fused stage tail: " + L2.name + " does not follow " + L.name);
+                b.t_Cout = L2.Cout; b.t_CoutPad = L2.CoutPad; b.t_w = L2.w->dev; b.t_epi = L2.bn->affine; b.t_slope = L2.slope;
+                b.t_sN = tail->out.sN; b.t_sC = tail->out.sC; b.t_sH = tail->out.sH;
+            } else {
+                const LSTMMod& M = *tail->M;
+                VR_CHECK(M.squeeze.Cin == L.Cout, -3, "fused LSTM squeeze: " + M.squeeze.name + " does not follow " + L.name);
+                b.t_Cout = 1; b.t_CoutPad = 1; b.t_w = M.squeeze.w->dev; b.t_epi = M.squeeze.bn->affine; b.t_slope = 0.f;
+                b.t_sN = (long long)a.Hout * a.Wout; b.t_sC = 0; b.t_sH = a.Wout;
+            }
+            const bool any_up = a.src[0].up || (a.nsrc > 1 && a.src[1].up) || (a.nsrc > 2 && a.src[2].up);
+            const bool by_rule = !(tail->kind == 2 && xt.MT == 64 && any_up);
+            if (by_rule && x3h_tail_ok(b, xt)) {
+                a.tail = b.tail; a.t_p = b.t_p; a.t_Cout = b.t_Cout; a.t_CoutPad = b.t_CoutPad; a.t_w = b.t_w; a.t_epi = b.t_epi;
+                a.t_slope = b.t_slope; a.t_sN = b.t_sN; a.t_sC = b.t_sC; a.t_sH = b.t_sH;
+                tail->done = true;
+                fused_tag = tail->kind == 1 ? "+tail" : "+squeeze";
+            }
+        }
+    }
     if (!dry && conv_sink) {
         PendingConv pc{};
         pc.a = a; pc.shp = shp;
@@ -842,7 +874,7 @@
         record_begin(0, flops);
         if (profiling) {
             char tag[160];
-            snprintf(tag, sizeof tag, "%s k%d s%d d%d ci%d co%d %dx%dx%d", L.name.c_str(), L.KS, L.stride, L.dh, L.Cin,
+            snprintf(tag, sizeof tag, "%s%s k%d s%d d%d ci%d co%d %dx%dx%d", L.name.c_str(), fused_tag, L.KS, L.stride, L.dh, L.Cin,
                      L.Cout, a.N, a.Hout, a.Wout);
             double bytes = conv_alg_bytes(L, a, N, batch_as_h);
             if (wcols < a.Wout) {
@@ -875,13 +907,12 @@
     return o;
 }
 
-Tensor Model::run_lstm(LSTMMod& M, const Tensor& h) {
+Tensor Model::run_lstm(LSTMMod& M, const Tensor& h, float* z, bool squeezed) {
     const int N = h.N, nb = h.H, nf = h.W;
     VR_CHECK(nb == M.nin, -2, "LSTM input size does not match the number of bins at dec2");
-    float* z = ws.allocf((size_t)N * nb * nf);
     const int nblk = launch_squeeze_conv(h, M.squeeze.w->dev, z, nullptr, true, stream);
     float* part = training ? ws.allocf((size_t)nblk * 2) : nullptr;
-    if (!dry) {
+    if (!dry && !squeezed) {
         launch_squeeze_conv(h, M.squeeze.w->dev, z, part, false, stream, training ? nullptr : M.squeeze.bn->affine);
         if (training) {
             BN* b = M.squeeze.bn;
@@ -958,7 +989,7 @@
     return SrcSpec{u};
 }
 
-Tensor Model::run_basenet(BaseNetL& B, const std::vector<SrcSpec>& in, int N, const Tensor* out_view) {
+Tensor Model::run_basenet(BaseNetL& B, const std::vector<SrcSpec>& in, int N, const Tensor* out_view, FusedTail* tail) {
     const std::string& p = B.prefix;
     Tensor e[5];
     e[0] = run_conv(B.enc1, in, N, nullptr, nullptr, false);
@@ -1063,9 +1094,12 @@
         if (taping()) tape.back().out.post = h.post;
     }
     tap(p + ".aspp", h);
+    FusedTail sq;
+    sq.kind = 2; sq.M = &B.lstm;
     for (int i = 0; i < 3; ++i) {
         SrcSpec up = upsampled(h);
-        h = run_conv(B.dec[i], {up, SrcSpec{e[3 - i]}}, N, nullptr, nullptr, false);
+        if (i == 2) sq.out.p = ws.allocf((size_t)N * e[1].H * e[1].W);
+        h = run_conv(B.dec[i], {up, SrcSpec{e[3 - i]}}, N, nullptr, nullptr, false, i == 2 ? &sq : nullptr);
         tap(p + ".dec" + std::to_string(4 - i), h);
     }
     static const bool lstm_fork = !getenv("VR_NO_LSTM_FORK");
@@ -1083,7 +1117,7 @@
         VR_HIP(hipEventRecord(lstm_join, side_stream));
         stream = ms;
     }
-    Tensor l = run_lstm(B.lstm, h);
+    Tensor l = run_lstm(B.lstm, h, sq.out.p, sq.done);
     tap(p + ".lstm", l);
     if (fk) VR_HIP(hipStreamWaitEvent(stream, lstm_join, 0));
     else uh = upsampled(h);
@@ -1091,7 +1125,7 @@
     const bool win = &B == &nets_[4] && net_w_hi > 0;
     if (win) { conv_w_lo = net_w_lo; conv_w_hi = net_w_hi; }
     Tensor o;
-    try { o = run_conv(B.dec[3], {uh, ul, SrcSpec{e[0]}}, N, out_view, nullptr, false); } catch (...) { conv_w_lo = conv_w_hi = 0; throw; }
+    try { o = run_conv(B.dec[3], {uh, ul, SrcSpec{e[0]}}, N, out_view, nullptr, false, tail); } catch (...) { conv_w_lo = conv_w_hi = 0; throw; }
     conv_w_lo = conv_w_hi = 0;
     tap(p + ".dec1", o);
     return o;
@@ -1128,12 +1162,21 @@
         VR_HIP(hipStreamWaitEvent(side_stream, ef, 0));
         band_fork_active = true;
     }
-    Tensor l1r = run_basenet(nets_[0], {SrcSpec{xl}}, B, nullptr);
+    auto low_band = [&](BaseNetL& net, Conv& tl, const std::vector<SrcSpec>& in, const Tensor& view) {
+        FusedTail ft;
+        ft.kind = 1; ft.L = &tl; ft.out = view; ft.out.C = tl.Cout;
+        Tensor r = run_basenet(net, in, B, nullptr, &ft);
+        if (!ft.done) return run_conv(tl, {SrcSpec{r}}, B, &view, nullptr, false);
+        Tensor o;
+        o.N = B; o.C = tl.Cout; o.H = view.H; o.W = view.W;
+        o.p = view.p; o.g = view.g; o.sN = view.sN; o.sC = view.sC; o.sH = view.sH;
+        o.aff0 = nullptr; o.slope = 1.f;
+        return o;
+    };
     v = half(aux1, 0);
-    Tensor l1 = run_conv(tail1, {SrcSpec{l1r}}, B, &v, nullptr, false);
-    Tensor l2r = run_basenet(nets_[2], {SrcSpec{xl}, SrcSpec{l1}}, B, nullptr);
+    Tensor l1 = low_band(nets_[0], tail1, {SrcSpec{xl}}, v);
     v = half(aux2, 0);
-    Tensor l2 = run_conv(tail2, {SrcSpec{l2r}}, B, &v, nullptr, false);
+    Tensor l2 = low_band(nets_[2], tail2, {SrcSpec{xl}, SrcSpec{l1}}, v);
     if (fork) stream = side_stream;
     const size_t tape_hi0 = tape.size();
     v = half(aux1, 1);
diff --git a/vocal-remover_amd/csrc/vr_common.h b/vocal-remover_amd/csrc/vr_common.h
--- a/vocal-remover_amd/csrc/vr_common.h
+++ b/vocal-remover_amd/csrc/vr_common.h
@@ -127,6 +127,13 @@
     int tapmask;
     int w_lo, w_hi;
     int wt0;
+    int tail;
+    int t_Cout, t_CoutPad;
+    const float* t_w;
+    const float* t_epi;
+    float t_slope;
+    float* t_p;
+    long long t_sN, t_sC, t_sH;
 };
 
 struct ConvShape {
```

After: 192,500 spectrogram-frames/sec (median of 6 runs). 2.2% higher.
